# XiaRho/MADM

Hardware: NVIDIA B200
Metric: UNet feature-extract images/s @512^2 (VAE-enc + q-sample + SD-1.4 UNet+LoRA taps + projections) (higher is better)
Workload: dtype fp16

## Files before the change

### include/madm_b200.h

```cpp
#ifndef MADM_B200_H_
#define MADM_B200_H_

#include <stddef.h>
#include <stdint.h>

#ifdef __cplusplus
extern "C" {
#endif

#define MADM_VERSION 100

enum {
  MADM_OK = 0,
  MADM_EINVAL = -1,
  MADM_ENOTFOUND = -2,
  MADM_ECUDA = -3,
  MADM_ESTATE = -4,
  MADM_ENOMEM = -5
};

#define MADM_DTYPE_BF16 0
#define MADM_DTYPE_FP16 1

typedef struct madm_ctx madm_ctx;
typedef void* madm_stream;

typedef struct madm_tensor {
  const char* name;
  const void* data;
  int32_t ndim;
  int64_t shape[4];
} madm_tensor;

int madm_version(void);
const char* madm_last_error(const madm_ctx* ctx);

int madm_create(madm_ctx** out, int device);
int madm_destroy(madm_ctx* ctx);

int madm_set_compute_dtype(madm_ctx* ctx, int32_t dtype);
int madm_get_compute_dtype(const madm_ctx* ctx);

#define MADM_VARIANT_BASE 0
#define MADM_VARIANT_S0 1
int madm_set_variant(madm_ctx* ctx, int32_t variant);
int madm_get_variant(const madm_ctx* ctx);

int madm_set_tensors(madm_ctx* ctx, const madm_tensor* named, int32_t n);

size_t madm_packed_bytes(madm_ctx* ctx);

int madm_pack_weights(madm_ctx* ctx, void* packed, const char* adapter, float lora_alpha_over_r, int32_t lora_only,
                      madm_stream stream);

#define MADM_STAGE_VAE 1
#define MADM_STAGE_UNET 2
#define MADM_STAGE_PROJ 4
#define MADM_STAGE_ALL 7
#define MADM_STAGE_HEAD 8
#define MADM_STAGE_DEC 16
#define MADM_STAGE_ALL_S0 23

size_t madm_workspace_bytes(madm_ctx* ctx, int32_t B);
size_t madm_workspace_bytes_head(madm_ctx* ctx, int32_t B, int32_t head_h, int32_t head_w);

#define MADM_FLAG_IMG_NORMALISED 1
#define MADM_FLAG_OUT_FP16 4
typedef struct madm_extract_args {
  int32_t B;
  int32_t stages;
  int32_t ema;
  int32_t flags;
  const float* img;
  const float* cond_inputs;
  const float* cond_emb;
  const int64_t* timesteps;
  const float* shared_noise;
  const float* noisy_latents_in;
  float* out[4];
  float* latents;
  float* noisy_latents;
  float* taps[4];
  const void* packed;
  void* workspace;
  size_t workspace_bytes;
  int32_t* range_flag;
  float* logits;
  float* unet_sample;
  float* decoded;
  float* decoded_raw;
  int32_t head_h, head_w;
  const void* packed_dgrad;
  const char* train_adapter;
  float train_lora_scale;
  float train_loss_scale;
} madm_extract_args;

int madm_extract(madm_ctx* ctx, const madm_extract_args* args, madm_stream stream);

#define MADM_KIND_GEMM 0
#define MADM_KIND_ATTENTION 1
#define MADM_KIND_GROUPNORM 2
#define MADM_KIND_LAYERNORM 3
#define MADM_KIND_ELEMENTWISE 4
#define MADM_NUM_KINDS 5
typedef struct madm_profile {
  struct { char name[32]; int32_t launches; double ms; double flops; double bytes; double exec_flops; } kind[MADM_NUM_KINDS];
} madm_profile;
int madm_set_profiling(madm_ctx* ctx, int32_t on);
int madm_get_profile(madm_ctx* ctx, madm_profile* out);
int madm_get_profile_stages(madm_ctx* ctx, int32_t stage_mask, madm_profile* out);

int madm_launch_count(madm_ctx* ctx, int32_t B, int32_t stages);

typedef struct madm_gemm_seg {
  const void* a;
  int32_t Bt, H, W, C, ld, ntaps;
  int8_t dx[9], dy[9];
  int32_t b_off[9];
} madm_gemm_seg;

typedef struct madm_gemm_args {
  madm_gemm_seg seg[2];
  int32_t nseg, M, N, Nw, ldw;
  const void* w;
  const float* bias;
  const float* rowbias;
  int32_t rows_per_img, ld_rowbias;
  const float* residual;
  int32_t ldr;
  float* out_f32; int32_t ldo32;
  void* out_bf16; int32_t ldo16;
  int32_t act;
  float alpha;
  int32_t bn;
  int32_t dtype;
  float* colstats;
  int32_t stat_rows;
  int32_t mt;
  int32_t s2d_H, s2d_W;
  int32_t pair;
  int32_t res16;
} madm_gemm_args;

int madm_op_gemm(const madm_gemm_args* a, madm_stream stream);
int madm_op_groupnorm(const void* x0, int32_t C0, const void* x1, int32_t C1, int32_t B, int32_t HW,
                      int32_t in16 , const float* gamma,
                      const float* beta, float eps, int32_t act, float* stats_scratch ,
                      void* y_bf16, void* raw_bf16, int32_t dtype, madm_stream stream);
int madm_op_groupnorm_from_colstats(const void* x, int32_t C, int32_t B, int32_t HW, int32_t in16, const float* colstats,
                                    int32_t stat_rows, const float* gamma, const float* beta, float eps, int32_t act,
                                    float* scratch , void* y_bf16, int32_t dtype, madm_stream stream);
int madm_op_groupnorm_scratch_floats(int32_t B, int32_t HW, int32_t C);
int madm_op_layernorm(const void* x, int32_t in16 , int32_t M, int32_t C, const float* gamma,
                      const float* beta, float eps, void* y_bf16, int32_t dtype, madm_stream stream);
int madm_op_softmax_rows(const float* s, int32_t R, int32_t L, void* p_bf16, int32_t dtype, madm_stream stream);
int madm_op_attention(const void* q, int32_t ldq, const void* k, int32_t ldk, const void* v, int32_t ldv, void* o, int32_t ldo,
                      int32_t B, int32_t heads, int32_t d, int32_t Nq, int32_t Nk, int64_t q_bstride, int64_t kv_bstride,
                      int64_t o_bstride, float scale, int32_t dtype, int32_t impl ,
                      madm_stream stream);
int madm_op_pack_linear(const float* w, int32_t N, int32_t K, const float* lora_a, const float* lora_b, int32_t r, float scale,
                        void* out_bf16, int32_t ldo, int32_t dtype, madm_stream stream);
int madm_op_pack_conv(const float* w, int32_t N, int32_t C, int32_t taps, int32_t Cpad, void* out_bf16, int32_t ldo,
                      int32_t dtype, madm_stream stream);
int madm_op_pack_conv_dgrad(const float* w, int32_t Cout, int32_t Cin, int32_t taps, int32_t CoPad, void* out_bf16, int32_t ldo, int32_t dtype,
                            madm_stream stream);
int madm_op_pack_linear_dgrad(const float* w, int32_t N, int32_t K, const float* lora_a, const float* lora_b, int32_t r, float scale,
                              void* out_bf16, int32_t ldo, int32_t dtype, madm_stream stream);
int madm_op_pack_geglu(const float* w, const float* bias, int32_t C4, int32_t K, void* out_bf16, float* out_bias,
                       int32_t dtype, madm_stream stream);
int madm_op_space_to_depth(const float* x, int32_t B, int32_t H, int32_t W, int32_t C, void* out_bf16, int32_t dtype,
                           madm_stream stream);
int madm_op_nchw_to_nhwc16(const float* x, int32_t B, int32_t C, int32_t HW, void* out16, int32_t dtype, madm_stream stream);
int madm_op_bilinear_resize(const void* src16, int32_t B, int32_t Hs, int32_t Ws, int32_t C, void* dst16, int32_t Hd, int32_t Wd,
                            int32_t dst_pitch, int32_t dtype, madm_stream stream);
int madm_op_depthwise3x3(const void* src16, int32_t B, int32_t H, int32_t W, int32_t C, int32_t dilation, const float* w9 ,
                         const float* shift , void* dst16, int32_t dtype, madm_stream stream);
int madm_op_pseudo_labels(const float* logits , int32_t B, int32_t C, int32_t h, int32_t w, int32_t H, int32_t W, float threshold,
                          int32_t ignore_top, int64_t* label , float* prob , float* weight ,
                          int32_t* count , madm_stream stream);
int madm_op_class_mask(const int64_t* label, int64_t n, const int64_t* classes, int32_t k, int64_t* mask, madm_stream stream);
int madm_op_one_mix(const int64_t* mask, int64_t n, const int64_t* label_a, const int64_t* label_b, int64_t* label_out ,
                    const float* weight_a, const float* weight_b, float* weight_out , madm_stream stream);
int madm_op_preprocess_image(const float* src , int32_t planes, int32_t Hs, int32_t Ws, int32_t Hr, int32_t Wr, int32_t Hd,
                             int32_t Wd, float* dst , madm_stream stream);
int madm_op_image_mix(const int64_t* mask , const float* a , const float* b, int32_t C, int64_t HW, float* out,
                      madm_stream stream);
int madm_op_color_jitter(const float* in, int32_t B, int64_t HW, const int32_t* order, const float* factors, const float* mean, const float* stdv,
                         float* out, madm_stream stream);
int madm_op_gaussian_blur(const float* src , int32_t planes, int32_t H, int32_t W, int32_t ky, int32_t kx, float sigma_y,
                          float sigma_x, float* tmp , float* dst, madm_stream stream);
int madm_op_ema_update(float* const* ema, const float* const* param, const int64_t* numel, int32_t n, float alpha, float one_minus_alpha,
                       madm_stream stream);
int madm_op_grad_norm_scratch_floats(int32_t n);
int madm_op_grad_norm(const float* const* grad, const int64_t* numel, int32_t n, float* scratch, float* out_norm, madm_stream stream);
int madm_op_adamw_step(float* const* param, const float* const* grad, float* const* exp_avg, float* const* exp_avg_sq, const int64_t* numel,
                       int32_t n, double lr, double beta1, double beta2, double eps, double weight_decay, int32_t step, const float* grad_norm,
                       float max_norm, madm_stream stream);
int madm_op_slide_merge(const float* feats, int32_t nwin, int32_t n, int32_t C, int32_t hf, int32_t wf, const int32_t* wins, int32_t Hf,
                        int32_t Wf, float* out, madm_stream stream);
int madm_op_upsample2x(const float* x, int32_t B, int32_t H, int32_t W, int32_t C, void* out_bf16, int32_t dtype,
                       madm_stream stream);
int madm_op_image_im2col(const float* img, int32_t B, int32_t H, int32_t W, void* out_bf16, int32_t* range_flag,
                         int32_t dtype, madm_stream stream);
int madm_op_gn_add_relu_nchw(const float* a, const float* ga, const float* ba, const float* s, const float* gs, const float* bs,
                             int32_t has_shortcut_norm, float eps, int32_t B, int32_t HW, int32_t C, float* stats_scratch,
                             float* out_nchw, madm_stream stream);

#define MADM_FLAG_TRAIN 2
int madm_set_grad_tensors(madm_ctx* ctx, const madm_tensor* named, int32_t n);
size_t madm_dgrad_packed_bytes(madm_ctx* ctx);
int madm_pack_dgrad_weights(madm_ctx* ctx, void* packed_dgrad, const char* adapter, float lora_alpha_over_r, int32_t trainable_only,
                            madm_stream stream);
size_t madm_train_workspace_bytes(madm_ctx* ctx, int32_t B, const char* adapter);
typedef struct madm_backward_args {
  int32_t B;
  int32_t reserved;
  const float* dout[4];
  const float* out[4];
  const float* cond_emb;
  float* d_cond_inputs;
  float* d_cond_emb;
  const char* adapter;
  float lora_alpha_over_r;
  float loss_scale;
  const void* packed;
  const void* packed_dgrad;
  void* workspace;
  size_t workspace_bytes;
} madm_backward_args;
int madm_backward(madm_ctx* ctx, const madm_backward_args* args, madm_stream stream);
int madm_backward_launch_count(madm_ctx* ctx, int32_t B);

int madm_op_groupnorm_bwd_scratch_floats(int32_t B, int32_t HW, int32_t C);
int madm_op_groupnorm_bwd(const void* x0, int32_t C0, const void* x1, int32_t C1, int32_t B, int32_t HW, int32_t in16, const float* stats,
                          const float* gamma, const float* beta, float eps, int32_t act, const void* dy16, const float* extra, float* scratch,
                          void* out16, float* dx0, int32_t acc0, float* dx1, int32_t acc1, float* dgamma, float* dbeta, int32_t dtype,
                          madm_stream stream);
int madm_op_layernorm_bwd(const float* x, int32_t M, int32_t C, const float* gamma, float eps, const void* dy16, float* dx, int32_t accumulate,
                          int32_t dtype, madm_stream stream);
int madm_op_geglu_fwd(const void* raw16, int64_t M, int32_t H, void* out16, int32_t dtype, madm_stream stream);
int madm_op_geglu_bwd(const void* raw16, const void* dout16, int64_t M, int32_t H, void* draw16, int32_t dtype, madm_stream stream);
int64_t madm_op_attention_bwd_scratch_floats(int32_t B, int32_t heads, int32_t d, int32_t Nq, int32_t Nk);
int madm_op_attention_bwd(const void* q, int32_t ldq, const void* k, int32_t ldk, const void* v, int32_t ldv, const void* o, int32_t ldo,
                          const void* dout, int32_t lddo, void* dq, int32_t lddq, void* dk, int32_t lddk, void* dv, int32_t lddv, int32_t B,
                          int32_t heads, int32_t d, int32_t Nq, int32_t Nk, int64_t q_bs, int64_t kv_bs, int64_t o_bs, int64_t do_bs, int64_t dq_bs,
                          int64_t dkv_bs, float scale, float* scratch, int32_t dtype, madm_stream stream);
int64_t madm_op_wgrad_scratch_floats(int32_t M, int32_t N, int32_t K, int32_t taps);
int madm_op_wgrad(const void* dy16, int32_t lda, const void* x16, int32_t ldb, int32_t M, int32_t N, int32_t K, int32_t taps, int32_t Bimg, int32_t H,
                  int32_t W, float alpha, float* out, int32_t transpose_out, float* scratch, int32_t dtype, madm_stream stream);
int64_t madm_op_lora_grads_scratch_floats(int32_t M, int32_t N, int32_t K);
int madm_op_lora_grads(const void* x16, int32_t ldx, const void* dy16, int32_t ldy, const void* a16, const void* bt16, int32_t M, int32_t N, int32_t K,
                       float alpha, float* gA, float* gB, float* scratch, int32_t dtype, madm_stream stream);
int madm_op_colsum_per_image(const void* x16, int32_t B, int32_t HW, int32_t C, float* out, int32_t ldo, int32_t dtype, madm_stream stream);
int madm_op_zero_stuff2x(const void* x16, int32_t B, int32_t h, int32_t w, int32_t C, void* out16, madm_stream stream);
int madm_op_sum2x2(const float* x, int32_t B, int32_t h, int32_t w, int32_t C, float* out, int32_t accumulate, madm_stream stream);
int madm_op_relu_bwd_nchw(const float* dout, const float* out, int32_t B, int32_t C, int32_t HW, float scale, void* dz16, int32_t dtype,
                          madm_stream stream);

#ifdef __cplusplus
}
#endif
#endif
```

### madm_b200/_lib.py

```python
import ctypes as C
import os
from typing import Optional

_HERE = os.path.dirname(os.path.abspath(__file__))
LIB_PATH = os.environ.get("MADM_B200_LIB") or os.path.join(_HERE, "libmadm_b200.so")

MADM_OK = 0
STAGE_VAE, STAGE_UNET, STAGE_PROJ, STAGE_ALL = 1, 2, 4, 7
STAGE_HEAD = 8
STAGE_DEC, STAGE_ALL_S0 = 16, 23
VARIANT_BASE, VARIANT_S0 = 0, 1
FLAG_IMG_NORMALISED = 1
FLAG_TRAIN = 2
FLAG_OUT_FP16 = 4
ACT_NONE, ACT_SILU, ACT_GEGLU, ACT_RELU = 0, 1, 2, 3
DTYPE_BF16, DTYPE_FP16 = 0, 1

c_void_p, c_int, c_int32, c_int64, c_float, c_size_t, c_char_p = (
    C.c_void_p, C.c_int, C.c_int32, C.c_int64, C.c_float, C.c_size_t, C.c_char_p)


class MadmTensor(C.Structure):
    _fields_ = [("name", c_char_p), ("data", c_void_p), ("ndim", c_int32), ("shape", c_int64 * 4)]


class MadmExtractArgs(C.Structure):
    _fields_ = [
        ("B", c_int32), ("stages", c_int32), ("ema", c_int32), ("flags", c_int32),
        ("img", c_void_p), ("cond_inputs", c_void_p), ("cond_emb", c_void_p), ("timesteps", c_void_p),
        ("shared_noise", c_void_p), ("noisy_latents_in", c_void_p),
        ("out", c_void_p * 4),
        ("latents", c_void_p), ("noisy_latents", c_void_p), ("taps", c_void_p * 4),
        ("packed", c_void_p), ("workspace", c_void_p), ("workspace_bytes", c_size_t),
        ("range_flag", c_void_p), ("logits", c_void_p),
        ("unet_sample", c_void_p), ("decoded", c_void_p), ("decoded_raw", c_void_p),
        ("head_h", c_int32), ("head_w", c_int32),
        ("packed_dgrad", c_void_p), ("train_adapter", c_char_p), ("train_lora_scale", c_float), ("train_loss_scale", c_float),
    ]


class MadmBackwardArgs(C.Structure):
    _fields_ = [
        ("B", c_int32), ("reserved", c_int32),
        ("dout", c_void_p * 4), ("out", c_void_p * 4), ("cond_emb", c_void_p),
        ("d_cond_inputs", c_void_p), ("d_cond_emb", c_void_p),
        ("adapter", c_char_p), ("lora_alpha_over_r", c_float), ("loss_scale", c_float),
        ("packed", c_void_p), ("packed_dgrad", c_void_p), ("workspace", c_void_p), ("workspace_bytes", c_size_t),
    ]


class _MadmProfileKind(C.Structure):
    _fields_ = [("name", C.c_char * 32), ("launches", c_int32), ("ms", C.c_double), ("flops", C.c_double), ("bytes", C.c_double),
                ("exec_flops", C.c_double)]


class MadmProfile(C.Structure):
    _fields_ = [("kind", _MadmProfileKind * 5)]


class MadmGemmSeg(C.Structure):
    _fields_ = [("a", c_void_p), ("Bt", c_int32), ("H", c_int32), ("W", c_int32), ("C", c_int32), ("ld", c_int32),
                ("ntaps", c_int32), ("dx", C.c_int8 * 9), ("dy", C.c_int8 * 9), ("b_off", c_int32 * 9)]


class MadmGemmArgs(C.Structure):
    _fields_ = [
        ("seg", MadmGemmSeg * 2), ("nseg", c_int32), ("M", c_int32), ("N", c_int32), ("Nw", c_int32), ("ldw", c_int32),
        ("w", c_void_p), ("bias", c_void_p), ("rowbias", c_void_p), ("rows_per_img", c_int32), ("ld_rowbias", c_int32),
        ("residual", c_void_p), ("ldr", c_int32), ("out_f32", c_void_p), ("ldo32", c_int32),
        ("out_bf16", c_void_p), ("ldo16", c_int32), ("act", c_int32), ("alpha", c_float), ("bn", c_int32), ("dtype", c_int32),
        ("colstats", c_void_p), ("stat_rows", c_int32), ("mt", c_int32), ("s2d_H", c_int32), ("s2d_W", c_int32), ("pair", c_int32), ("res16", c_int32),
    ]


SYMBOLS = {
    "madm_version": (c_int, []),
    "madm_last_error": (c_char_p, [c_void_p]),
    "madm_create": (c_int, [C.POINTER(c_void_p), c_int]),
    "madm_destroy": (c_int, [c_void_p]),
    "madm_set_compute_dtype": (c_int, [c_void_p, c_int32]),
    "madm_get_compute_dtype": (c_int, [c_void_p]),
    "madm_set_variant": (c_int, [c_void_p, c_int32]),
    "madm_get_variant": (c_int, [c_void_p]),
    "madm_set_tensors": (c_int, [c_void_p, C.POINTER(MadmTensor), c_int32]),
    "madm_packed_bytes": (c_size_t, [c_void_p]),
    "madm_pack_weights": (c_int, [c_void_p, c_void_p, c_char_p, c_float, c_int32, c_void_p]),
    "madm_workspace_bytes": (c_size_t, [c_void_p, c_int32]),
    "madm_workspace_bytes_head": (c_size_t, [c_void_p, c_int32, c_int32, c_int32]),
    "madm_extract": (c_int, [c_void_p, C.POINTER(MadmExtractArgs), c_void_p]),
    "madm_set_grad_tensors": (c_int, [c_void_p, C.POINTER(MadmTensor), c_int32]),
    "madm_dgrad_packed_bytes": (c_size_t, [c_void_p]),
    "madm_pack_dgrad_weights": (c_int, [c_void_p, c_void_p, c_char_p, c_float, c_int32, c_void_p]),
    "madm_train_workspace_bytes": (c_size_t, [c_void_p, c_int32, c_char_p]),
    "madm_backward": (c_int, [c_void_p, C.POINTER(MadmBackwardArgs), c_void_p]),
    "madm_backward_launch_count": (c_int, [c_void_p, c_int32]),
    "madm_launch_count": (c_int, [c_void_p, c_int32, c_int32]),
    "madm_set_profiling": (c_int, [c_void_p, c_int32]),
    "madm_get_profile": (c_int, [c_void_p, C.POINTER(MadmProfile)]),
    "madm_get_profile_stages": (c_int, [c_void_p, c_int32, C.POINTER(MadmProfile)]),
    "madm_op_gemm": (c_int, [C.POINTER(MadmGemmArgs), c_void_p]),
    "madm_op_groupnorm": (c_int, [c_void_p, c_int32, c_void_p, c_int32, c_int32, c_int32, c_int32, c_void_p, c_void_p, c_float,
                                  c_int32, c_void_p, c_void_p, c_void_p, c_int32, c_void_p]),
    "madm_op_groupnorm_scratch_floats": (c_int, [c_int32, c_int32, c_int32]),
    "madm_op_groupnorm_from_colstats": (c_int, [c_void_p, c_int32, c_int32, c_int32, c_int32, c_void_p, c_int32, c_void_p, c_void_p,
                                                c_float, c_int32, c_void_p, c_void_p, c_int32, c_void_p]),
    "madm_op_layernorm": (c_int, [c_void_p, c_int32, c_int32, c_int32, c_void_p, c_void_p, c_float, c_void_p, c_int32, c_void_p]),
    "madm_op_softmax_rows": (c_int, [c_void_p, c_int32, c_int32, c_void_p, c_int32, c_void_p]),
    "madm_op_attention": (c_int, [c_void_p, c_int32, c_void_p, c_int32, c_void_p, c_int32, c_void_p, c_int32, c_int32,
                                  c_int32, c_int32, c_int32, c_int32, c_int64, c_int64, c_int64, c_float, c_int32, c_int32, c_void_p]),
    "madm_op_pack_linear": (c_int, [c_void_p, c_int32, c_int32, c_void_p, c_void_p, c_int32, c_float, c_void_p, c_int32,
                                    c_int32, c_void_p]),
    "madm_op_pack_conv": (c_int, [c_void_p, c_int32, c_int32, c_int32, c_int32, c_void_p, c_int32, c_int32, c_void_p]),
    "madm_op_pack_conv_dgrad": (c_int, [c_void_p, c_int32, c_int32, c_int32, c_int32, c_void_p, c_int32, c_int32, c_void_p]),
    "madm_op_pack_linear_dgrad": (c_int, [c_void_p, c_int32, c_int32, c_void_p, c_void_p, c_int32, c_float, c_void_p, c_int32, c_int32, c_void_p]),
    "madm_op_pack_geglu": (c_int, [c_void_p, c_void_p, c_int32, c_int32, c_void_p, c_void_p, c_int32, c_void_p]),
    "madm_op_space_to_depth": (c_int, [c_void_p, c_int32, c_int32, c_int32, c_int32, c_void_p, c_int32, c_void_p]),
    "madm_op_nchw_to_nhwc16": (c_int, [c_void_p, c_int32, c_int32, c_int32, c_void_p, c_int32, c_void_p]),
    "madm_op_bilinear_resize": (c_int, [c_void_p, c_int32, c_int32, c_int32, c_int32, c_void_p, c_int32, c_int32, c_int32, c_int32, c_void_p]),
    "madm_op_depthwise3x3": (c_int, [c_void_p, c_int32, c_int32, c_int32, c_int32, c_int32, c_void_p, c_void_p, c_void_p, c_int32, c_void_p]),
    "madm_op_pseudo_labels": (c_int, [c_void_p, c_int32, c_int32, c_int32, c_int32, c_int32, c_int32, c_float, c_int32, c_void_p, c_void_p,
                                      c_void_p, c_void_p, c_void_p]),
    "madm_op_class_mask": (c_int, [c_void_p, c_int64, c_void_p, c_int32, c_void_p, c_void_p]),
    "madm_op_one_mix": (c_int, [c_void_p, c_int64, c_void_p, c_void_p, c_void_p, c_void_p, c_void_p, c_void_p, c_void_p]),
    "madm_op_preprocess_image": (c_int, [c_void_p, c_int32, c_int32, c_int32, c_int32, c_int32, c_int32, c_int32, c_void_p, c_void_p]),
    "madm_op_image_mix": (c_int, [c_void_p, c_void_p, c_void_p, c_int32, c_int64, c_void_p, c_void_p]),
    "madm_op_color_jitter": (c_int, [c_void_p, c_int32, c_int64, c_void_p, c_void_p, c_void_p, c_void_p, c_void_p, c_void_p]),
    "madm_op_gaussian_blur": (c_int, [c_void_p, c_int32, c_int32, c_int32, c_int32, c_int32, c_float, c_float, c_void_p, c_void_p, c_void_p]),
    "madm_op_ema_update": (c_int, [c_void_p, c_void_p, c_void_p, c_int32, c_float, c_float, c_void_p]),
    "madm_op_grad_norm_scratch_floats": (c_int, [c_int32]),
    "madm_op_grad_norm": (c_int, [c_void_p, c_void_p, c_int32, c_void_p, c_void_p, c_void_p]),
    "madm_op_adamw_step": (c_int, [c_void_p, c_void_p, c_void_p, c_void_p, c_void_p, c_int32, C.c_double, C.c_double, C.c_double, C.c_double,
                                   C.c_double, c_int32, c_void_p, c_float, c_void_p]),
    "madm_op_slide_merge": (c_int, [c_void_p, c_int32, c_int32, c_int32, c_int32, c_int32, c_void_p, c_int32, c_int32, c_void_p, c_void_p]),
    "madm_op_upsample2x": (c_int, [c_void_p, c_int32, c_int32, c_int32, c_int32, c_void_p, c_int32, c_void_p]),
    "madm_op_image_im2col": (c_int, [c_void_p, c_int32, c_int32, c_int32, c_void_p, c_void_p, c_int32, c_void_p]),
    "madm_op_groupnorm_bwd_scratch_floats": (c_int, [c_int32, c_int32, c_int32]),
    "madm_op_groupnorm_bwd": (c_int, [c_void_p, c_int32, c_void_p, c_int32, c_int32, c_int32, c_int32, c_void_p, c_void_p, c_void_p, c_float, c_int32,
                                      c_void_p, c_void_p, c_void_p, c_void_p, c_void_p, c_int32, c_void_p, c_int32, c_void_p, c_void_p, c_int32, c_void_p]),
    "madm_op_layernorm_bwd": (c_int, [c_void_p, c_int32, c_int32, c_void_p, c_float, c_void_p, c_void_p, c_int32, c_int32, c_void_p]),
    "madm_op_geglu_fwd": (c_int, [c_void_p, c_int64, c_int32, c_void_p, c_int32, c_void_p]),
    "madm_op_geglu_bwd": (c_int, [c_void_p, c_void_p, c_int64, c_int32, c_void_p, c_int32, c_void_p]),
    "madm_op_attention_bwd_scratch_floats": (c_int64, [c_int32, c_int32, c_int32, c_int32, c_int32]),
    "madm_op_attention_bwd": (c_int, [c_void_p, c_int32, c_void_p, c_int32, c_void_p, c_int32, c_void_p, c_int32, c_void_p, c_int32, c_void_p, c_int32,
                                      c_void_p, c_int32, c_void_p, c_int32, c_int32, c_int32, c_int32, c_int32, c_int32, c_int64, c_int64, c_int64,
                                      c_int64, c_int64, c_int64, c_float, c_void_p, c_int32, c_void_p]),
    "madm_op_wgrad_scratch_floats": (c_int64, [c_int32, c_int32, c_int32, c_int32]),
    "madm_op_wgrad": (c_int, [c_void_p, c_int32, c_void_p, c_int32, c_int32, c_int32, c_int32, c_int32, c_int32, c_int32, c_int32, c_float, c_void_p,
                              c_int32, c_void_p, c_int32, c_void_p]),
    "madm_op_lora_grads_scratch_floats": (c_int64, [c_int32, c_int32, c_int32]),
    "madm_op_lora_grads": (c_int, [c_void_p, c_int32, c_void_p, c_int32, c_void_p, c_void_p, c_int32, c_int32, c_int32, c_float, c_void_p, c_void_p,
                                   c_void_p, c_int32, c_void_p]),
    "madm_op_colsum_per_image": (c_int, [c_void_p, c_int32, c_int32, c_int32, c_void_p, c_int32, c_int32, c_void_p]),
    "madm_op_zero_stuff2x": (c_int, [c_void_p, c_int32, c_int32, c_int32, c_int32, c_void_p, c_void_p]),
    "madm_op_sum2x2": (c_int, [c_void_p, c_int32, c_int32, c_int32, c_int32, c_void_p, c_int32, c_void_p]),
    "madm_op_relu_bwd_nchw": (c_int, [c_void_p, c_void_p, c_int32, c_int32, c_int32, c_float, c_void_p, c_int32, c_void_p]),
    "madm_op_gn_add_relu_nchw": (c_int, [c_void_p, c_void_p, c_void_p, c_void_p, c_void_p, c_void_p, c_int32, c_float,
                                         c_int32, c_int32, c_int32, c_void_p, c_void_p, c_void_p]),
}

_lib: Optional[C.CDLL] = None


class MadmError(RuntimeError):
    pass


def load() -> C.CDLL:
    global _lib
    if _lib is not None:
        return _lib
    if not os.path.exists(LIB_PATH):
        raise MadmError(
            f"{LIB_PATH} not found: build it with `python -c 'import __graft_entry__ as g; g.build()'` "
            "(nvcc, sm_100a). madm_b200 has no CPU / PyTorch fallback.")
    lib = C.CDLL(LIB_PATH)
    for name, (res, args) in SYMBOLS.items():
        fn = getattr(lib, name)
        fn.restype = res
        fn.argtypes = args
    _lib = lib
    return lib


def check(rc: int, ctx=None, what: str = ""):
    if rc != MADM_OK:
        lib = load()
        msg = lib.madm_last_error(ctx)
        raise MadmError(f"{what} failed ({rc}): {msg.decode() if msg else ''}")
```

### madm_b200/csrc/api_ops.cu

```cuda
#include "../../include/madm_b200.h"
#include "api_internal.h"
#include "kernels.h"

#include <string.h>

using namespace madm;

namespace madm {
static thread_local char g_err[512] = "";
void set_global_error(const char* msg) {
  strncpy(g_err, msg ? msg : "", sizeof(g_err) - 1);
  g_err[sizeof(g_err) - 1] = 0;
}
const char* global_error() { return g_err; }
}

static int fail(const char* e) {
  set_global_error(e);
  return MADM_EINVAL;
}
#define RUN(expr)                      \
  do {                                 \
    const char* _e = (expr);           \
    if (_e) return fail(_e);           \
    return MADM_OK;                    \
  } while (0)

extern "C" {

int madm_op_gemm(const madm_gemm_args* a, madm_stream stream) {
  if (!a) return fail("madm_op_gemm: null args");
  GemmDesc d;
  d.nseg = a->nseg;
  for (int s = 0; s < 2; ++s) {
    const madm_gemm_seg& g = a->seg[s];
    GemmASeg& t = d.seg[s];
    t.ptr = g.a; t.Bt = g.Bt; t.H = g.H; t.W = g.W; t.C = g.C; t.ld = g.ld; t.ntaps = g.ntaps;
    for (int i = 0; i < 9; ++i) { t.dx[i] = g.dx[i]; t.dy[i] = g.dy[i]; t.b_off[i] = g.b_off[i]; }
  }
  d.M = a->M; d.N = a->N; d.w = a->w; d.Nw = a->Nw; d.ldw = a->ldw;
  d.bias = a->bias; d.rowbias = a->rowbias; d.rows_per_img = a->rows_per_img; d.ld_rowbias = a->ld_rowbias;
  d.residual = a->residual; d.ldr = a->ldr;
  d.out_f32 = a->out_f32; d.ldo32 = a->ldo32; d.out_bf16 = a->out_bf16; d.ldo16 = a->ldo16;
  d.act = a->act; d.alpha = a->alpha; d.bn = a->bn; d.fp16 = a->dtype == MADM_DTYPE_FP16;
  d.colstats = a->colstats; d.stat_rows = a->stat_rows ? a->stat_rows : 32; d.mt = a->mt; d.s2d_H = a->s2d_H; d.s2d_W = a->s2d_W; d.pair = a->pair; d.res16 = a->res16;
  GemmLaunch L;
  if (const char* e = gemm_prepare(d, &L)) return fail(e);
  RUN(gemm_launch(L, static_cast<cudaStream_t>(stream)));
}

int madm_op_groupnorm(const void* x0, int32_t C0, const void* x1, int32_t C1, int32_t B, int32_t HW, int32_t in16, const float* gamma,
                      const float* beta, float eps, int32_t act, float* stats, void* y, void* raw, int32_t dtype, madm_stream stream) {
  cudaStream_t st = static_cast<cudaStream_t>(stream);
  const int f16 = dtype == MADM_DTYPE_FP16;
  if (const char* e = groupnorm_stats(x0, C0, x1, C1, B, HW, in16, f16, stats, st)) return fail(e);
  RUN(groupnorm_apply(x0, C0, x1, C1, B, HW, in16, stats, 0, gamma, beta, eps, act, y, raw, f16, st));
}

int madm_op_layernorm(const void* x, int32_t in16, int32_t M, int32_t C, const float* gamma, const float* beta, float eps, void* y,
                      int32_t dtype, madm_stream stream) {
  RUN(layernorm(x, in16, M, C, gamma, beta, eps, y, dtype == MADM_DTYPE_FP16, static_cast<cudaStream_t>(stream)));
}

int madm_op_softmax_rows(const float* s, int32_t R, int32_t L, void* p, int32_t dtype, madm_stream stream) {
  RUN(softmax_rows(s, R, L, p, dtype == MADM_DTYPE_FP16, static_cast<cudaStream_t>(stream)));
}

int madm_op_attention(const void* q, int32_t ldq, const void* k, int32_t ldk, const void* v, int32_t ldv, void* o, int32_t ldo,
                      int32_t B, int32_t heads, int32_t d, int32_t Nq, int32_t Nk, int64_t q_bs, int64_t kv_bs, int64_t o_bs,
                      float scale, int32_t dtype, int32_t impl, madm_stream stream) {
  if (impl != 0) return fail("madm_op_attention: impl must be 0 (the mma.sync kernel of round 1 was removed from the library)");
  FaLaunch L;
  if (const char* e = flash_attention_tc_prepare(q, ldq, k, ldk, v, ldv, o, ldo, B, heads, d, Nq, Nk, q_bs, kv_bs, o_bs, scale,
                                                 dtype == MADM_DTYPE_FP16, &L))
    return fail(e);
  RUN(flash_attention_tc_launch(L, static_cast<cudaStream_t>(stream)));
}

int madm_op_pack_linear(const float* w, int32_t N, int32_t K, const float* la, const float* lb, int32_t r, float scale, void* out,
                        int32_t ldo, int32_t dtype, madm_stream stream) {
  RUN(pack_linear_weight(w, N, K, la, lb, r, scale, ldo ? ldo : K, out, dtype == MADM_DTYPE_FP16, static_cast<cudaStream_t>(stream)));
}

int madm_op_pack_conv(const float* w, int32_t N, int32_t C, int32_t taps, int32_t Cpad, void* out, int32_t ldo, int32_t dtype,
                      madm_stream stream) {
  const int Kpad = taps * Cpad;
  RUN(pack_conv_weight(w, N, C, taps, Cpad, Kpad, ldo ? ldo : Kpad, out, dtype == MADM_DTYPE_FP16, static_cast<cudaStream_t>(stream)));
}

int madm_op_pack_conv_dgrad(const float* w, int32_t Cout, int32_t Cin, int32_t taps, int32_t CoPad, void* out, int32_t ldo, int32_t dtype,
                            madm_stream stream) {
  const int Kpad = taps * CoPad;
  RUN(pack_conv_dgrad_weight(w, Cout, Cin, taps, CoPad, Kpad, ldo ? ldo : Kpad, out, dtype == MADM_DTYPE_FP16, static_cast<cudaStream_t>(stream)));
}

int madm_op_pack_linear_dgrad(const float* w, int32_t N, int32_t K, const float* lora_a, const float* lora_b, int32_t r, float scale, void* out,
                              int32_t ldo, int32_t dtype, madm_stream stream) {
  RUN(pack_linear_dgrad_weight(w, N, K, lora_a, lora_b, r, scale, ldo ? ldo : N, out, dtype == MADM_DTYPE_FP16, static_cast<cudaStream_t>(stream)));
}

int madm_op_pack_geglu(const float* w, const float* bias, int32_t C4, int32_t K, void* out, float* out_bias, int32_t dtype,
                       madm_stream stream) {
  RUN(pack_geglu_weight(w, bias, C4, K, out, out_bias, dtype == MADM_DTYPE_FP16, static_cast<cudaStream_t>(stream)));
}

int madm_op_space_to_depth(const float* x, int32_t B, int32_t H, int32_t W, int32_t C, void* out, int32_t dtype, madm_stream stream) {
  RUN(space_to_depth(x, B, H, W, C, out, dtype == MADM_DTYPE_FP16, static_cast<cudaStream_t>(stream)));
}

int madm_op_upsample2x(const float* x, int32_t B, int32_t H, int32_t W, int32_t C, void* out, int32_t dtype, madm_stream stream) {
  RUN(upsample_nearest2x(x, B, H, W, C, out, dtype == MADM_DTYPE_FP16, static_cast<cudaStream_t>(stream)));
}

int madm_op_nchw_to_nhwc16(const float* x, int32_t B, int32_t C, int32_t HW, void* out, int32_t dtype, madm_stream stream) {
  RUN(nchw_to_nhwc16(x, B, C, HW, out, dtype == MADM_DTYPE_FP16, static_cast<cudaStream_t>(stream)));
}

int madm_op_bilinear_resize(const void* src, int32_t B, int32_t Hs, int32_t Ws, int32_t C, void* dst, int32_t Hd, int32_t Wd, int32_t ldd,
                            int32_t dtype, madm_stream stream) {
  RUN(bilinear_resize_nhwc16(src, B, Hs, Ws, C, dst, Hd, Wd, ldd, dtype == MADM_DTYPE_FP16, static_cast<cudaStream_t>(stream)));
}

int madm_op_depthwise3x3(const void* src, int32_t B, int32_t H, int32_t W, int32_t C, int32_t dilation, const float* w9, const float* shift,
                         void* dst, int32_t dtype, madm_stream stream) {
  RUN(depthwise3x3_nhwc16(src, B, H, W, C, dilation, w9, shift, dst, dtype == MADM_DTYPE_FP16, static_cast<cudaStream_t>(stream)));
}

int madm_op_pseudo_labels(const float* logits, int32_t B, int32_t C, int32_t h, int32_t w, int32_t H, int32_t W, float threshold,
                          int32_t ignore_top, int64_t* label, float* prob, float* weight, int32_t* count, madm_stream stream) {
  RUN(pseudo_labels(logits, B, C, h, w, H, W, threshold, ignore_top, label, prob, weight, count, static_cast<cudaStream_t>(stream)));
}

int madm_op_class_mask(const int64_t* label, int64_t n, const int64_t* classes, int32_t k, int64_t* mask, madm_stream stream) {
  RUN(class_mask(label, long(n), classes, k, mask, static_cast<cudaStream_t>(stream)));
}

int madm_op_one_mix(const int64_t* mask, int64_t n, const int64_t* label_a, const int64_t* label_b, int64_t* label_out, const float* weight_a,
                    const float* weight_b, float* weight_out, madm_stream stream) {
  RUN(one_mix(mask, long(n), label_a, label_b, label_out, weight_a, weight_b, weight_out, static_cast<cudaStream_t>(stream)));
}

int madm_op_ema_update(float* const* ema, const float* const* param, const int64_t* numel, int32_t n, float alpha, float one_minus_alpha,
                       madm_stream stream) {
  if (!ema || !param || !numel || n < 1) return fail("madm_op_ema_update: null argument");
  RUN(ema_update(ema, param, reinterpret_cast<const long*>(numel), n, alpha, one_minus_alpha, static_cast<cudaStream_t>(stream)));
}

int madm_op_grad_norm_scratch_floats(int32_t n) { return grad_norm_scratch_floats(n); }

int madm_op_grad_norm(const float* const* grad, const int64_t* numel, int32_t n, float* scratch, float* out_norm, madm_stream stream) {
  if (!grad || !numel || !scratch || !out_norm || n < 1) return fail("madm_op_grad_norm: null argument");
  RUN(grad_norm(grad, reinterpret_cast<const long*>(numel), n, scratch, out_norm, static_cast<cudaStream_t>(stream)));
}

int madm_op_adamw_step(float* const* param, const float* const* grad, float* const* exp_avg, float* const* exp_avg_sq, const int64_t* numel,
                       int32_t n, double lr, double beta1, double beta2, double eps, double weight_decay, int32_t step, const float* grad_norm,
                       float max_norm, madm_stream stream) {
  if (!param || !grad || !exp_avg || !exp_avg_sq || !numel || n < 1) return fail("madm_op_adamw_step: null argument");
  RUN(adamw_step(param, grad, exp_avg, exp_avg_sq, reinterpret_cast<const long*>(numel), n, lr, beta1, beta2, eps, weight_decay, step, grad_norm,
                 max_norm, static_cast<cudaStream_t>(stream)));
}

int madm_op_preprocess_image(const float* src, int32_t planes, int32_t Hs, int32_t Ws, int32_t Hr, int32_t Wr, int32_t Hd, int32_t Wd, float* dst,
                             madm_stream stream) {
  if (!src || !dst) return fail("madm_op_preprocess_image: null argument");
  RUN(resize_bilinear_nchw(src, planes, Hs, Ws, Hr, Wr, Hd, Wd, dst, static_cast<cudaStream_t>(stream)));
}

int madm_op_image_mix(const int64_t* mask, const float* a, const float* b, int32_t C, int64_t HW, float* out, madm_stream stream) {
  if (!mask || !a || !b || !out) return fail("madm_op_image_mix: null argument");
  RUN(image_mix(mask, a, b, C, long(HW), out, static_cast<cudaStream_t>(stream)));
}

int madm_op_color_jitter(const float* in, int32_t B, int64_t HW, const int32_t* order, const float* factors, const float* mean, const float* stdv,
                         float* out, madm_stream stream) {
  if (!in || !order || !factors || !out) return fail("madm_op_color_jitter: null argument");
  RUN(color_jitter(in, B, long(HW), order, factors, mean, stdv, out, static_cast<cudaStream_t>(stream)));
}

int madm_op_gaussian_blur(const float* src, int32_t planes, int32_t H, int32_t W, int32_t ky, int32_t kx, float sigma_y, float sigma_x, float* tmp,
                          float* dst, madm_stream stream) {
  if (!src || !tmp || !dst) return fail("madm_op_gaussian_blur: null argument");
  RUN(gaussian_blur(src, planes, H, W, ky, kx, sigma_y, sigma_x, tmp, dst, static_cast<cudaStream_t>(stream)));
}

int madm_op_slide_merge(const float* feats, int32_t nwin, int32_t n, int32_t C, int32_t hf, int32_t wf, const int32_t* wins, int32_t Hf, int32_t Wf,
                        float* out, madm_stream stream) {
  RUN(slide_merge(feats, nwin, n, C, hf, wf, wins, Hf, Wf, out, static_cast<cudaStream_t>(stream)));
}

int madm_op_image_im2col(const float* img, int32_t B, int32_t H, int32_t W, void* out, int32_t* range_flag, int32_t dtype,
                         madm_stream stream) {
  RUN(image_im2col(img, B, H, W, out, range_flag, dtype == MADM_DTYPE_FP16, static_cast<cudaStream_t>(stream)));
}

int madm_op_groupnorm_from_colstats(const void* x, int32_t C, int32_t B, int32_t HW, int32_t in16, const float* colstats, int32_t stat_rows,
                                    const float* gamma, const float* beta, float eps, int32_t act, float* scratch , void* y,
                                    int32_t dtype, madm_stream stream) {
  cudaStream_t st = static_cast<cudaStream_t>(stream);
  const int f16 = dtype == MADM_DTYPE_FP16;
  if (HW % stat_rows != 0) return fail("groupnorm_from_colstats: HW must be a multiple of stat_rows");
  if (stat_rows != 32) return fail("groupnorm_from_colstats: stat_rows must be 32");
  const int nb = HW / stat_rows;
  if (const char* e = groupnorm_colstats_reduce(colstats, C, nullptr, 0, B, nb, scratch, st)) return fail(e);
  RUN(groupnorm_apply(x, C, nullptr, 0, B, HW, in16, scratch, groupnorm_colstats_chunks(nb), gamma, beta, eps, act, y, nullptr, f16, st));
}

int madm_op_groupnorm_scratch_floats(int32_t B, int32_t HW, int32_t C) {
  return int(size_t(2) * B * groupnorm_slabs(HW, C) * 64 + size_t(2) * B * 64);
}

int madm_op_gn_add_relu_nchw(const float* a, const float* ga, const float* ba, const float* s, const float* gs, const float* bs,
                             int32_t has_shortcut_norm, float eps, int32_t B, int32_t HW, int32_t C, float* stats, float* out,
                             madm_stream stream) {
  cudaStream_t st = static_cast<cudaStream_t>(stream);
  const size_t per = size_t(B) * groupnorm_slabs(HW, C) * 64;
  float* pa = stats;
  float* ps = stats + per;
  float* st_a = stats + 2 * per;
  float* st_s = st_a + size_t(B) * 64;
  if (const char* e = groupnorm_stats(a, C, nullptr, 0, B, HW, 0, 0, pa, st)) return fail(e);
  if (const char* e = groupnorm_finalize(pa, B, HW, C, st_a, st)) return fail(e);
  if (has_shortcut_norm) {
    if (const char* e = groupnorm_stats(s, C, nullptr, 0, B, HW, 0, 0, ps, st)) return fail(e);
    if (const char* e = groupnorm_finalize(ps, B, HW, C, st_s, st)) return fail(e);
  }
  RUN(gn_add_relu_nchw(a, st_a, ga, ba, s, has_shortcut_norm ? st_s : nullptr, gs, bs, eps, B, HW, C, out, st));
}

int madm_op_groupnorm_bwd_scratch_floats(int32_t B, int32_t HW, int32_t C) {
  return int(size_t(B) * groupnorm_bwd_slabs(HW) * C * 2 + size_t(B) * 64 + size_t(B) * C * 2);
}
int madm_op_groupnorm_bwd(const void* x0, int32_t C0, const void* x1, int32_t C1, int32_t B, int32_t HW, int32_t in16, const float* stats,
                          const float* gamma, const float* beta, float eps, int32_t act, const void* dy16, const float* extra, float* scratch,
                          void* out16, float* dx0, int32_t acc0, float* dx1, int32_t acc1, float* dgamma, float* dbeta, int32_t dtype,
                          madm_stream stream) {
  const int C = C0 + C1;
  float* partial = scratch;
  float* coef = partial + size_t(B) * groupnorm_bwd_slabs(HW) * C * 2;
  float* chan = coef + size_t(B) * 64;
  RUN(groupnorm_bwd(x0, C0, x1, C1, B, HW, in16, stats, gamma, beta, eps, act, dy16, dtype == MADM_DTYPE_FP16, partial, coef, chan, extra, out16, dx0,
                    acc0, dx1, acc1, dgamma, dbeta, 1.0f, static_cast<cudaStream_t>(stream)));
}
int madm_op_layernorm_bwd(const float* x, int32_t M, int32_t C, const float* gamma, float eps, const void* dy16, float* dx, int32_t accumulate,
                          int32_t dtype, madm_stream stream) {
  RUN(layernorm_bwd(x, M, C, gamma, eps, dy16, dtype == MADM_DTYPE_FP16, dx, accumulate, static_cast<cudaStream_t>(stream)));
}
int madm_op_geglu_fwd(const void* raw16, int64_t M, int32_t H, void* out16, int32_t dtype, madm_stream stream) {
  RUN(geglu_fwd(raw16, long(M), H, out16, dtype == MADM_DTYPE_FP16, static_cast<cudaStream_t>(stream)));
}
int madm_op_geglu_bwd(const void* raw16, const void* dout16, int64_t M, int32_t H, void* draw16, int32_t dtype, madm_stream stream) {
  RUN(geglu_bwd(raw16, dout16, long(M), H, draw16, dtype == MADM_DTYPE_FP16, static_cast<cudaStream_t>(stream)));
}
int64_t madm_op_attention_bwd_scratch_floats(int32_t B, int32_t heads, int32_t d, int32_t Nq, int32_t Nk) {
  return int64_t(attention_bwd_scratch_floats(B, heads, d, Nq, Nk));
}
int madm_op_attention_bwd(const void* q, int32_t ldq, const void* k, int32_t ldk, const void* v, int32_t ldv, const void* o, int32_t ldo,
                          const void* dout, int32_t lddo, void* dq, int32_t lddq, void* dk, int32_t lddk, void* dv, int32_t lddv, int32_t B,
                          int32_t heads, int32_t d, int32_t Nq, int32_t Nk, int64_t q_bs, int64_t kv_bs, int64_t o_bs, int64_t do_bs, int64_t dq_bs,
                          int64_t dkv_bs, float scale, float* scratch, int32_t dtype, madm_stream stream) {
  RUN(attention_bwd(q, ldq, k, ldk, v, ldv, o, ldo, dout, lddo, dq, lddq, dk, lddk, dv, lddv, B, heads, d, Nq, Nk, long(q_bs), long(kv_bs), long(kv_bs),
                    long(o_bs), long(do_bs), long(dq_bs), long(dkv_bs), long(dkv_bs), scale, scratch, dtype == MADM_DTYPE_FP16,
                    static_cast<cudaStream_t>(stream)));
}
int64_t madm_op_wgrad_scratch_floats(int32_t M, int32_t N, int32_t K, int32_t taps) { return int64_t(wgrad_scratch_floats(M, N, K, taps)); }
int madm_op_wgrad(const void* dy16, int32_t lda, const void* x16, int32_t ldb, int32_t M, int32_t N, int32_t K, int32_t taps, int32_t Bimg, int32_t H,
                  int32_t W, float alpha, float* out, int32_t transpose_out, float* scratch, int32_t dtype, madm_stream stream) {
  long so_n = K, so_k = 1, so_tap = 0;
  if (taps == 9) { so_n = long(K) * 9; so_k = 9; so_tap = 1; }
  else if (transpose_out) { so_n = 1; so_k = N; }
  RUN(wgrad(dy16, lda, x16, ldb, M, N, K, taps, Bimg, H, W, alpha, out, so_n, so_k, so_tap, scratch, dtype == MADM_DTYPE_FP16,
            static_cast<cudaStream_t>(stream)));
}
int64_t madm_op_lora_grads_scratch_floats(int32_t M, int32_t N, int32_t K) { return lora_grads_supported(N, K) ? int64_t(lora_grads_scratch_floats(M, N, K)) : -1; }
int madm_op_lora_grads(const void* x16, int32_t ldx, const void* dy16, int32_t ldy, const void* a16, const void* bt16, int32_t M, int32_t N, int32_t K,
                       float alpha, float* gA, float* gB, float* scratch, int32_t dtype, madm_stream stream) {
  RUN(lora_grads(x16, ldx, dy16, ldy, a16, bt16, M, N, K, alpha, gA, gB, scratch, dtype == MADM_DTYPE_FP16, static_cast<cudaStream_t>(stream)));
}
int madm_op_colsum_per_image(const void* x16, int32_t B, int32_t HW, int32_t C, float* out, int32_t ldo, int32_t dtype, madm_stream stream) {
  RUN(colsum_per_image(x16, B, HW, C, dtype == MADM_DTYPE_FP16, out, ldo, static_cast<cudaStream_t>(stream)));
}
int madm_op_zero_stuff2x(const void* x16, int32_t B, int32_t h, int32_t w, int32_t C, void* out16, madm_stream stream) {
  RUN(zero_stuff2x(x16, B, h, w, C, out16, static_cast<cudaStream_t>(stream)));
}
int madm_op_sum2x2(const float* x, int32_t B, int32_t h, int32_t w, int32_t C, float* out, int32_t accumulate, madm_stream stream) {
  RUN(sum2x2(x, B, h, w, C, out, accumulate, static_cast<cudaStream_t>(stream)));
}
int madm_op_relu_bwd_nchw(const float* dout, const float* out, int32_t B, int32_t C, int32_t HW, float scale, void* dz16, int32_t dtype,
                          madm_stream stream) {
  RUN(relu_bwd_nchw_to_nhwc16(dout, out, B, C, HW, scale, dz16, dtype == MADM_DTYPE_FP16, static_cast<cudaStream_t>(stream)));
}

}
```

### madm_b200/csrc/attention_tc.cu

```cuda
#include "cvt.cuh"
#include "kernels.h"
#include "launch.cuh"
#include "ptx.cuh"

#include <mutex>
#include <stdio.h>

namespace madm {

static constexpr int FA_BM = 128;
static constexpr int FA_BN = 128;
static constexpr int FA_TILE = 128 * 128;

template <int D, int NQT>
struct FaCfg {
  static constexpr int KC = (D + 63) / 64;
  static constexpr int DV = (D + 15) / 16 * 16;
  static constexpr int KSTEPS = (D + 15) / 16;
  static constexpr bool REG_S = D <= 80;
  static constexpr bool ONES = REG_S && DV > D;
  static constexpr int NSB = REG_S ? 1 : 2;
  static constexpr bool P_TMEM = ONES && NQT == 2;
  static constexpr int Q_BYTES = NQT * KC * FA_TILE;
  static constexpr int KV_BYTES = KC * FA_TILE;
  static constexpr int P_BYTES = P_TMEM ? 0 : NQT * 2 * FA_TILE;
  static constexpr int STAGES = (Q_BYTES + P_BYTES + 4 * KV_BYTES + 2048 <= 227 * 1024) ? 2 : 1;
  static constexpr size_t SMEM = Q_BYTES + 2 * STAGES * KV_BYTES + P_BYTES + 1024 + 512;
  static constexpr int S_COLS = NQT * NSB * 128;
  static constexpr int P_COLS = P_TMEM ? NQT * 64 : 0;
  static constexpr int O_BASE = S_COLS + P_COLS;
  static constexpr int O_STRIDE = (DV + 31) / 32 * 32;
  static constexpr int TMEM_NEED = O_BASE + NQT * O_STRIDE;
  static constexpr int TMEM_COLS = TMEM_NEED <= 256 ? 256 : 512;
  static constexpr int THREADS = 32 * (1 + NQT) + NQT * 128;
  static_assert(TMEM_NEED <= 512, "TMEM budget");
  static_assert(SMEM <= 227 * 1024, "smem budget");
};

struct FaParams {
  CUtensorMap tmQ, tmK, tmV;
  uint16_t* O;
  int ldo;
  long o_bs;
  int Nq, Nk;
  float scale_log2;
  int fp16;
  float* lse;
};

__device__ __forceinline__ float fa_ex2(float x) {
  float y;
  asm("ex2.approx.ftz.f32 %0, %1;" : "=f"(y) : "f"(x));
  return y;
}

template <int D, int NQT, bool FP16>
__global__ void __launch_bounds__(FaCfg<D, NQT>::THREADS, 1) fa_tc_kernel(const __grid_constant__ FaParams p) {
  using C = FaCfg<D, NQT>;
  extern __shared__ uint8_t smem_raw[];
  const uint32_t base = (smem_u32(smem_raw) + 1023u) & ~1023u;
  const uint32_t sQ = base;
  const uint32_t sK = sQ + C::Q_BYTES;
  const uint32_t sV = sK + C::STAGES * C::KV_BYTES;
  const uint32_t sP = sV + C::STAGES * C::KV_BYTES;
  const uint32_t sBar = sP + C::P_BYTES;
  const uint32_t q_full = sBar;
  auto k_full = [&](int s) { return sBar + 8u * (1 + s); };
  auto k_empty = [&](int s) { return sBar + 8u * (3 + s); };
  auto v_full = [&](int s) { return sBar + 8u * (5 + s); };
  auto v_empty = [&](int s) { return sBar + 8u * (7 + s); };
  auto gbar = [&](int g, int i) { return sBar + 8u * (9 + g * 8 + i); };
  auto s_full = [&](int g, int a) { return gbar(g, a); };
  auto s_empty = [&](int g, int a) { return gbar(g, 2 + a); };
  auto pv_go = [&](int g) { return gbar(g, 4); };
  auto pv_done = [&](int g) { return gbar(g, 5); };
  const uint32_t tmem_slot = sBar + 8u * (9 + 16);
  volatile uint32_t* tmem_slot_ptr = reinterpret_cast<volatile uint32_t*>(smem_raw + (tmem_slot - smem_u32(smem_raw)));

  const int warp = threadIdx.x >> 5, lane = threadIdx.x & 31;
  const int q0 = blockIdx.x * (FA_BM * NQT), h = blockIdx.y, b = blockIdx.z;
  const int ntiles = (p.Nk + FA_BN - 1) / FA_BN;

  if (warp == 0 && lane == 0) {
    prefetch_tmap(&p.tmQ); prefetch_tmap(&p.tmK); prefetch_tmap(&p.tmV);
    mbar_init(q_full, 1);
    for (int s = 0; s < 2; ++s) {
      mbar_init(k_full(s), 1); mbar_init(k_empty(s), NQT); mbar_init(v_full(s), 1); mbar_init(v_empty(s), NQT);
    }
    for (int g = 0; g < NQT; ++g) {
      for (int a = 0; a < 2; ++a) { mbar_init(s_full(g, a), 1); mbar_init(s_empty(g, a), 4); }
      mbar_init(pv_go(g), 4); mbar_init(pv_done(g), 1);
    }
    fence_mbar_init();
  }
  if (warp == 1) {
    tmem_alloc(tmem_slot, C::TMEM_COLS);
    tmem_relinquish();
  }
  tc_fence_before();
  __syncthreads();
  tc_fence_after();
  const uint32_t tmem = *tmem_slot_ptr;
  pdl_trigger();
  pdl_wait();

  if (warp == 0) {
    if (elect_one()) {
      mbar_arrive_expect_tx(q_full, C::Q_BYTES);
#pragma unroll
      for (int g = 0; g < NQT; ++g)
#pragma unroll
        for (int kc = 0; kc < C::KC; ++kc)
          tma_load_4d(sQ + (g * C::KC + kc) * FA_TILE, &p.tmQ, q_full, kc * 64, h, q0 + g * FA_BM, b);
      int stage = 0;
      uint32_t phase = 0;
      for (int j = 0; j < ntiles; ++j) {
        mbar_wait(k_empty(stage), phase ^ 1u);
        mbar_arrive_expect_tx(k_full(stage), C::KV_BYTES);
#pragma unroll
        for (int kc = 0; kc < C::KC; ++kc) tma_load_4d(sK + stage * C::KV_BYTES + kc * FA_TILE, &p.tmK, k_full(stage), kc * 64, h, j * FA_BN, b);
        mbar_wait(v_empty(stage), phase ^ 1u);
        mbar_arrive_expect_tx(v_full(stage), C::KV_BYTES);
#pragma unroll
        for (int kc = 0; kc < C::KC; ++kc) tma_load_4d(sV + stage * C::KV_BYTES + kc * FA_TILE, &p.tmV, v_full(stage), kc * 64, h, j * FA_BN, b);
        if (++stage == C::STAGES) { stage = 0; phase ^= 1u; }
      }
    }
  } else if (warp <= NQT) {
    if (elect_one()) {
      const int g = warp - 1;
      const uint32_t idesc_s = make_idesc_16(FA_BM, FA_BN, FP16 ? 1 : 0);
      const uint32_t idesc_o = make_idesc_16(FA_BM, C::DV, FP16 ? 1 : 0) | (1u << 16);
      uint64_t qd[C::KSTEPS], kd[C::STAGES][C::KSTEPS], vd[C::STAGES], pd[2];
#pragma unroll
      for (int ks = 0; ks < C::KSTEPS; ++ks) {
        const int kc = ks >> 2, k = ks & 3;
        qd[ks] = make_smem_desc_sw128(sQ + (g * C::KC + kc) * FA_TILE) + uint64_t(2 * k);
#pragma unroll
        for (int st = 0; st < C::STAGES; ++st) kd[st][ks] = make_smem_desc_sw128(sK + st * C::KV_BYTES + kc * FA_TILE) + uint64_t(2 * k);
      }
#pragma unroll
      for (int st = 0; st < C::STAGES; ++st) vd[st] = make_smem_desc_sw128_mn(sV + st * C::KV_BYTES, FA_TILE);
      pd[0] = make_smem_desc_sw128(sP + (g * 2) * FA_TILE);
      pd[1] = make_smem_desc_sw128(sP + (g * 2 + 1) * FA_TILE);
      const uint32_t tmem_og = tmem + C::O_BASE + g * C::O_STRIDE;
      const uint32_t tmem_pg = tmem + C::S_COLS + g * 64;
      auto issue_s = [&](int j) {
        const int stage = j % C::STAGES;
        const int sb = j % C::NSB;
        mbar_wait(k_full(stage), (j / C::STAGES) & 1);
        mbar_wait(s_empty(g, sb), ((j / C::NSB) & 1) ^ 1u);
        tc_fence_after();
        const uint32_t ts = tmem + uint32_t((g * C::NSB + sb) * 128);
#pragma unroll
        for (int ks = 0; ks < C::KSTEPS; ++ks) umma_bf16_ss(ts, qd[ks], stage == 0 ? kd[0][ks] : kd[C::STAGES - 1][ks], idesc_s, ks != 0);
        umma_commit(s_full(g, sb));
        umma_commit(k_empty(stage));
      };
      mbar_wait(q_full, 0);
      issue_s(0);
      for (int j = 0; j < ntiles; ++j) {
        if (j + 1 < ntiles) issue_s(j + 1);
        const int stage = j % C::STAGES;
        int keys = p.Nk - j * FA_BN;
        if (keys > FA_BN) keys = FA_BN;
        const int ksteps = (keys + 15) >> 4;
        mbar_wait(pv_go(g), j & 1);
        tc_fence_after();
        const uint64_t vds = stage == 0 ? vd[0] : vd[C::STAGES - 1];
#pragma unroll
        for (int kk = 0; kk < FA_BN / 16; ++kk) {
          if (kk < ksteps) {
            const uint64_t bd = vds + uint64_t(kk * (2048 >> 4));
            if constexpr (C::P_TMEM) umma_f16_ts(tmem_og, tmem_pg + kk * 8, bd, idesc_o, kk != 0);
            else umma_bf16_ss(tmem_og, pd[kk >> 2] + uint64_t(2 * (kk & 3)), bd, idesc_o, kk != 0);
          }
        }
        umma_commit(pv_done(g));
        umma_commit(v_empty(stage));
      }
    }
  } else {
    const int g = (warp - (1 + NQT)) >> 2;
    const int q = warp & 3;
    const int row = q * 32 + lane;
    const uint32_t lane_base = uint32_t(q * 32) << 16;
    const uint32_t sPg = sP + uint32_t(g * 2) * FA_TILE;
    const uint32_t tmem_o = tmem + lane_base + C::O_BASE + g * C::O_STRIDE;
    const uint32_t tmem_p = tmem + lane_base + C::S_COLS + g * 64;
    const float sl = p.scale_log2;
    constexpr int fp16 = FP16 ? 1 : 0;
    constexpr int OC = C::ONES ? D + 1 : D;
    float o_acc[C::DV];
#pragma unroll
    for (int i = 0; i < C::DV; ++i) o_acc[i] = 0.f;
    float m_run = -INFINITY, l_run = 0.f, corr_prev = 1.f;
    uint32_t r[32];

    auto o_update = [&](float corr) {
      tc_fence_after();
      constexpr int OB = (C::DV % 48 == 0) ? 48 : 32;
#pragma unroll
      for (int c0 = 0; c0 < C::DV; c0 += OB) {
        uint32_t ro[OB];
        __syncwarp();
        if (c0 + 0 < C::DV) tmem_ld16_at<0>(tmem_o + c0, ro);
        if (c0 + 16 < C::DV) tmem_ld16_at<16>(tmem_o + c0 + 16, ro);
        if constexpr (OB == 48) { if (c0 + 32 < C::DV) tmem_ld16_at<32>(tmem_o + c0 + 32, ro); }
        tmem_ld_wait();
#pragma unroll
        for (int i = 0; i < OB; ++i)
          if (c0 + i < OC) o_acc[c0 + i] = fmaf(o_acc[c0 + i], corr, __uint_as_float(ro[i]));
      }
      tc_fence_before();
    };

    for (int j = 0; j < ntiles; ++j) {
      const int sb = j % C::NSB;
      mbar_wait(s_full(g, sb), (j / C::NSB) & 1);
      tc_fence_after();
      const uint32_t ts = tmem + lane_base + uint32_t((g * C::NSB + sb) * 128);
      const int kvalid = p.Nk - j * FA_BN;
      const bool ragged = kvalid < FA_BN;
      float corr, rs = 0.f;
      if constexpr (C::REG_S && C::P_TMEM) {
        uint32_t sc[4][32];
        __syncwarp();
#pragma unroll
        for (int c = 0; c < 4; ++c) tmem_ld32(ts + c * 32, sc[c]);
        tmem_ld_wait();
        tc_fence_before();
        __syncwarp();
        if (lane == 0) mbar_arrive(s_empty(g, sb));
        if (ragged) {
#pragma unroll
          for (int c = 0; c < 4; ++c)
#pragma unroll
            for (int i = 0; i < 32; ++i)
              if (c * 32 + i >= kvalid) sc[c][i] = 0xff800000u;
        }
        float mx0 = m_run, mx1 = -INFINITY, mx2 = -INFINITY, mx3 = -INFINITY;
#pragma unroll
        for (int i = 0; i < 32; ++i) {
          mx0 = fmaxf(mx0, __uint_as_float(sc[0][i]));
          mx1 = fmaxf(mx1, __uint_as_float(sc[1][i]));
          mx2 = fmaxf(mx2, __uint_as_float(sc[2][i]));
          mx3 = fmaxf(mx3, __uint_as_float(sc[3][i]));
        }
        const float mx = fmaxf(fmaxf(mx0, mx1), fmaxf(mx2, mx3));
        corr = fa_ex2((m_run - mx) * sl);
        m_run = mx;
        const float ms = -mx * sl;
        {
          const int stage = j % C::STAGES;
          mbar_wait(v_full(stage), (j / C::STAGES) & 1);
          if constexpr (C::ONES) {
            const uint32_t addr = sV + stage * C::KV_BYTES + uint32_t(D >> 6) * FA_TILE + uint32_t(row) * 128 +
                                  uint32_t((((D & 63) >> 3) ^ (row & 7)) << 4) + uint32_t((D & 7) * 2);
            const uint16_t one = FP16 ? 0x3C00 : 0x3F80;
            asm volatile("st.shared.u16 [%0], %1;" ::"r"(addr), "h"(one) : "memory");
          }
        }
        float rs1 = 0.f;
#pragma unroll
        for (int c = 0; c < 4; ++c) {
          uint32_t pk[16];
#pragma unroll
          for (int i = 0; i < 32; i += 2) {
            const float p0 = fa_ex2(fmaf(__uint_as_float(sc[c][i]), sl, ms));
            const float p1 = fa_ex2(fmaf(__uint_as_float(sc[c][i + 1]), sl, ms));
            pk[i >> 1] = pack2_16(p0, p1, fp16);
            if constexpr (!C::ONES) { rs += p0; rs1 += p1; }
          }
          if (c == 0) {
            if (j > 0) mbar_wait(pv_done(g), (j - 1) & 1);
            if constexpr (C::P_TMEM) { tc_fence_after(); __syncwarp(); }
          }
          if constexpr (C::P_TMEM) {
            tmem_st16(tmem_p + c * 16, pk);
          } else {
            const uint32_t chunk_base = sPg + uint32_t(c >> 1) * FA_TILE + uint32_t(row) * 128;
            const int u0 = (c & 1) * 4;
#pragma unroll
            for (int u = 0; u < 4; ++u) {
              const uint32_t addr = chunk_base + uint32_t(((u0 + u) ^ (row & 7)) << 4);
              asm volatile("st.shared.v4.b32 [%0], {%1,%2,%3,%4};" ::"r"(addr), "r"(pk[4 * u]), "r"(pk[4 * u + 1]), "r"(pk[4 * u + 2]),
                           "r"(pk[4 * u + 3]) : "memory");
            }
          }
        }
        if constexpr (C::P_TMEM) { tmem_st_wait(); tc_fence_before(); }
        rs += rs1;
      } else if constexpr (C::REG_S) {
        uint32_t sa[32], sb2[32];
        float mx0 = m_run, mx1 = -INFINITY, mx2 = -INFINITY, mx3 = -INFINITY;
#pragma unroll
        for (int hlf = 0; hlf < 2; ++hlf) {
          __syncwarp();
          tmem_ld32(ts + hlf * 64, sa);
          tmem_ld32(ts + hlf * 64 + 32, sb2);
          tmem_ld_wait();
          if (ragged) {
#pragma unroll
            for (int i = 0; i < 32; ++i) {
              if (hlf * 64 + i >= kvalid) sa[i] = 0xff800000u;
              if (hlf * 64 + 32 + i >= kvalid) sb2[i] = 0xff800000u;
            }
          }
#pragma unroll
          for (int i = 0; i < 32; i += 2) {
            mx0 = fmaxf(mx0, __uint_as_float(sa[i]));
            mx1 = fmaxf(mx1, __uint_as_float(sa[i + 1]));
            mx2 = fmaxf(mx2, __uint_as_float(sb2[i]));
            mx3 = fmaxf(mx3, __uint_as_float(sb2[i + 1]));
          }
        }
        const float mx = fmaxf(fmaxf(mx0, mx1), fmaxf(mx2, mx3));
        corr = fa_ex2((m_run - mx) * sl);
        m_run = mx;
        const float ms = -mx * sl;
        {
          const int stage = j % C::STAGES;
          mbar_wait(v_full(stage), (j / C::STAGES) & 1);
          if constexpr (C::ONES) {
            const uint32_t addr = sV + stage * C::KV_BYTES + uint32_t(D >> 6) * FA_TILE + uint32_t(row) * 128 +
                                  uint32_t((((D & 63) >> 3) ^ (row & 7)) << 4) + uint32_t((D & 7) * 2);
            const uint16_t one = FP16 ? 0x3C00 : 0x3F80;
            asm volatile("st.shared.u16 [%0], %1;" ::"r"(addr), "h"(one) : "memory");
          }
        }
        float rs1 = 0.f;
        __syncwarp();
        tmem_ld32(ts, sa);
#pragma unroll
        for (int c = 0; c < 4; ++c) {
          uint32_t (&cur)[32] = (c & 1) ? sb2 : sa;
          uint32_t (&nxt)[32] = (c & 1) ? sa : sb2;
          tmem_ld_wait();
          if (c < 3) {
            __syncwarp();
            tmem_ld32(ts + (c + 1) * 32, nxt);
          } else {
            tc_fence_before();
            __syncwarp();
            if (lane == 0) mbar_arrive(s_empty(g, sb));
          }
          if (ragged) {
#pragma unroll
            for (int i = 0; i < 32; ++i)
              if (c * 32 + i >= kvalid) cur[i] = 0xff800000u;
          }
          uint32_t pk[16];
#pragma unroll
          for (int i = 0; i < 32; i += 2) {
            const float p0 = fa_ex2(fmaf(__uint_as_float(cur[i]), sl, ms));
            const float p1 = fa_ex2(fmaf(__uint_as_float(cur[i + 1]), sl, ms));
            pk[i >> 1] = pack2_16(p0, p1, fp16);
            if constexpr (!C::ONES) { rs += p0; rs1 += p1; }
          }
          if (c == 0 && j > 0) mbar_wait(pv_done(g), (j - 1) & 1);
          const uint32_t chunk_base = sPg + uint32_t(c >> 1) * FA_TILE + uint32_t(row) * 128;
          const int u0 = (c & 1) * 4;
#pragma unroll
          for (int u = 0; u < 4; ++u) {
            const uint32_t addr = chunk_base + uint32_t(((u0 + u) ^ (row & 7)) << 4);
            asm volatile("st.shared.v4.b32 [%0], {%1,%2,%3,%4};" ::"r"(addr), "r"(pk[4 * u]), "r"(pk[4 * u + 1]), "r"(pk[4 * u + 2]),
                         "r"(pk[4 * u + 3]) : "memory");
          }
        }
        rs += rs1;
      } else {
        float mx = m_run;
#pragma unroll 1
        for (int c = 0; c < FA_BN; c += 32) {
          __syncwarp();
          tmem_ld32(ts + c, r);
          tmem_ld_wait();
          if (c + 32 <= kvalid) {
#pragma unroll
            for (int i = 0; i < 32; ++i) mx = fmaxf(mx, __uint_as_float(r[i]));
          } else {
#pragma unroll
            for (int i = 0; i < 32; ++i)
              if (c + i < kvalid) mx = fmaxf(mx, __uint_as_float(r[i]));
          }
        }
        corr = fa_ex2((m_run - mx) * sl);
        m_run = mx;
        const float ms = -mx * sl;
        mbar_wait(v_full(j % C::STAGES), (j / C::STAGES) & 1);
        if (j > 0) mbar_wait(pv_done(g), (j - 1) & 1);
#pragma unroll 1
        for (int c = 0; c < FA_BN; c += 32) {
          __syncwarp();
          tmem_ld32(ts + c, r);
          tmem_ld_wait();
          uint32_t pk[16];
#pragma unroll
          for (int i = 0; i < 32; i += 2) {
            float p0 = fa_ex2(fmaf(__uint_as_float(r[i]), sl, ms));
            float p1 = fa_ex2(fmaf(__uint_as_float(r[i + 1]), sl, ms));
            if (c + i >= kvalid) p0 = 0.f;
            if (c + i + 1 >= kvalid) p1 = 0.f;
            rs += p0 + p1;
            pk[i >> 1] = pack2_16(p0, p1, fp16);
          }
          const uint32_t chunk_base = sPg + uint32_t(c >> 6) * FA_TILE + uint32_t(row) * 128;
          const int u0 = (c & 63) >> 3;
#pragma unroll
          for (int u = 0; u < 4; ++u) {
            const uint32_t addr = chunk_base + uint32_t(((u0 + u) ^ (row & 7)) << 4);
            asm volatile("st.shared.v4.b32 [%0], {%1,%2,%3,%4};" ::"r"(addr), "r"(pk[4 * u]), "r"(pk[4 * u + 1]), "r"(pk[4 * u + 2]),
                         "r"(pk[4 * u + 3]) : "memory");
          }
        }
        tc_fence_before();
        __syncwarp();
        if (lane == 0) mbar_arrive(s_empty(g, sb));
      }
      l_run = l_run * corr + rs;
      fence_proxy_async();
      if (j > 0) o_update(corr_prev);
      corr_prev = corr;
      tc_fence_before();
      __syncwarp();
      if (lane == 0) mbar_arrive(pv_go(g));
    }
    mbar_wait(pv_done(g), (ntiles - 1) & 1);
    o_update(corr_prev);
    const int m = q0 + g * FA_BM + row;
    if (m < p.Nq) {
      const float den = C::ONES ? o_acc[C::ONES ? D : 0] : l_run;
      const float inv = 1.0f / den;
      if (p.lse) p.lse[(size_t(b) * gridDim.y + h) * p.Nq + m] = (m_run * p.scale_log2 + log2f(den)) * 0.6931471805599453f;
      uint16_t* op = p.O + size_t(b) * p.o_bs + size_t(m) * p.ldo + h * D;
#pragma unroll
      for (int c = 0; c < D; c += 8) {
        uint4 v;
        v.x = pack2_16(o_acc[c] * inv, o_acc[c + 1] * inv, fp16);
        v.y = pack2_16(o_acc[c + 2] * inv, o_acc[c + 3] * inv, fp16);
        v.z = pack2_16(o_acc[c + 4] * inv, o_acc[c + 5] * inv, fp16);
        v.w = pack2_16(o_acc[c + 6] * inv, o_acc[c + 7] * inv, fp16);
        *reinterpret_cast<uint4*>(op + c) = v;
      }
    }
  }

  tc_fence_before();
  __syncthreads();
  if (warp == 1) {
    tc_fence_after();
    tmem_dealloc(tmem, C::TMEM_COLS);
  }
}

typedef CUresult (*EncodeTiledFn)(CUtensorMap*, CUtensorMapDataType, cuuint32_t, void*, const cuuint64_t*, const cuuint64_t*,
                                  const cuuint32_t*, const cuuint32_t*, CUtensorMapInterleave, CUtensorMapSwizzle,
                                  CUtensorMapL2promotion, CUtensorMapFloatOOBfill);
static EncodeTiledFn fa_encode_fn() {
  static EncodeTiledFn fn = nullptr;
  static std::once_flag once;
  std::call_once(once, [] {
    void* p = nullptr;
    cudaDriverEntryPointQueryResult qres;
    if (cudaGetDriverEntryPoint("cuTensorMapEncodeTiled", &p, cudaEnableDefault, &qres) == cudaSuccess && qres == cudaDriverEntryPointSuccess)
      fn = reinterpret_cast<EncodeTiledFn>(p);
  });
  return fn;
}

static const char* fa_map(CUtensorMap* tm, const void* ptr, int d, int heads, int ntok, int B, int ld, long bstride) {
  EncodeTiledFn fn = fa_encode_fn();
  if (!fn) return "cuTensorMapEncodeTiled unavailable";
  cuuint64_t dims[4] = {cuuint64_t(d), cuuint64_t(heads), cuuint64_t(ntok), cuuint64_t(B)};
  cuuint64_t strides[3] = {cuuint64_t(d) * 2, cuuint64_t(ld) * 2, cuuint64_t(bstride) * 2};
  if (B == 1) strides[2] = cuuint64_t(ntok) * ld * 2;
  cuuint32_t box[4] = {64, 1, 128, 1};
  cuuint32_t estr[4] = {1, 1, 1, 1};
  CUresult r = fn(tm, CU_TENSOR_MAP_DATA_TYPE_UINT16, 4, const_cast<void*>(ptr), dims, strides, box, estr, CU_TENSOR_MAP_INTERLEAVE_NONE,
                  CU_TENSOR_MAP_SWIZZLE_128B, CU_TENSOR_MAP_L2_PROMOTION_L2_256B, CU_TENSOR_MAP_FLOAT_OOB_FILL_NONE);
  if (r != CUDA_SUCCESS) {
    static thread_local char buf[128];
    snprintf(buf, sizeof(buf), "attention: cuTensorMapEncodeTiled failed (CUresult %d)", int(r));
    return buf;
  }
  return nullptr;
}

const char* flash_attention_tc_prepare(const void* q, int ldq, const void* k, int ldk, const void* v, int ldv, void* o, int ldo, int B,
                                       int heads, int d, int Nq, int Nk, long q_bs, long kv_bs, long o_bs, float scale, int fp16,
                                       FaLaunch* L, float* lse) {
  if (d != 40 && d != 80 && d != 160) return "attention: unsupported head dim (40, 80, 160)";
  if (ldq % 8 || ldk % 8 || ldv % 8 || ldo % 8 || q_bs % 8 || kv_bs % 8) return "attention: pitches must be multiples of 8 elements";
  if ((reinterpret_cast<uintptr_t>(q) | reinterpret_cast<uintptr_t>(k) | reinterpret_cast<uintptr_t>(v) | reinterpret_cast<uintptr_t>(o)) & 15)
    return "attention: pointers must be 16-byte aligned";
  if (Nq < 1 || Nk < 1) return "attention: empty problem";
  static_assert(sizeof(FaParams) <= sizeof(L->params), "FaLaunch::params too small");
  FaParams* p = reinterpret_cast<FaParams*>(L->params);
  if (const char* e = fa_map(&p->tmQ, q, d, heads, Nq, B, ldq, q_bs)) return e;
  if (const char* e = fa_map(&p->tmK, k, d, heads, Nk, B, ldk, kv_bs)) return e;
  if (const char* e = fa_map(&p->tmV, v, d, heads, Nk, B, ldv, kv_bs)) return e;
  p->O = reinterpret_cast<uint16_t*>(o);
  p->ldo = ldo; p->o_bs = o_bs; p->Nq = Nq; p->Nk = Nk;
  p->scale_log2 = scale * 1.4426950408889634f;
  p->fp16 = fp16;
  p->lse = lse;
  L->d = d;
  L->nqt = (d <= 80 && Nq >= 2 * FA_BM) ? 2 : 1;
  L->grid = dim3((Nq + FA_BM * L->nqt - 1) / (FA_BM * L->nqt), heads, B);
  return nullptr;
}

template <int D, int NQT, bool FP16>
static const char* fa_launch_t(const FaLaunch& L, cudaStream_t st) {
  using C = FaCfg<D, NQT>;
  static bool attr = false;
  if (!attr) {
    if (cudaFuncSetAttribute(fa_tc_kernel<D, NQT, FP16>, cudaFuncAttributeMaxDynamicSharedMemorySize, int(C::SMEM)) != cudaSuccess)
      return "attention: cudaFuncSetAttribute failed";
    attr = true;
  }
  if (launch_k(fa_tc_kernel<D, NQT, FP16>, L.grid, dim3(C::THREADS), C::SMEM, st, *reinterpret_cast<const FaParams*>(L.params)) != cudaSuccess)
    return "fa_tc launch failed";
  return cudaGetLastError() == cudaSuccess ? nullptr : "attention: launch failed";
}
template <int D, int NQT>
static const char* fa_launch_d(const FaLaunch& L, cudaStream_t st) {
  return reinterpret_cast<const FaParams*>(L.params)->fp16 ? fa_launch_t<D, NQT, true>(L, st) : fa_launch_t<D, NQT, false>(L, st);
}

const char* flash_attention_tc_launch(const FaLaunch& L, cudaStream_t st) {
  switch (L.d) {
    case 40: return L.nqt == 2 ? fa_launch_d<40, 2>(L, st) : fa_launch_d<40, 1>(L, st);
    case 80: return L.nqt == 2 ? fa_launch_d<80, 2>(L, st) : fa_launch_d<80, 1>(L, st);
    case 160: return fa_launch_d<160, 1>(L, st);
  }
  return "attention: unsupported head dim";
}

}
```

### madm_b200/ops.py

```python
import ctypes as C
from typing import Optional, Sequence

import torch

from . import _lib
from ._lib import MadmGemmArgs, MadmGemmSeg


def _ptr(t: Optional[torch.Tensor]):
    return None if t is None else C.c_void_p(t.data_ptr())


def _dt(dtype) -> int:
    if dtype == torch.float16:
        return _lib.DTYPE_FP16
    if dtype == torch.bfloat16:
        return _lib.DTYPE_BF16
    raise _lib.MadmError(f"operand dtype must be torch.float16 or torch.bfloat16, got {dtype}")


def _stream():
    return C.c_void_p(torch.cuda.current_stream().cuda_stream)


def taps_3x3():
    return [(kx - 1, ky - 1, 0) for ky in range(3) for kx in range(3)]


def taps_stride2(B: int, pad1: bool):
    out = []
    for ky in range(3):
        for kx in range(3):
            if pad1:
                py, dy = (0 if ky == 1 else 1), (-1 if ky == 0 else 0)
                px, dx = (0 if kx == 1 else 1), (-1 if kx == 0 else 0)
            else:
                py, dy = (1 if ky == 1 else 0), (1 if ky == 2 else 0)
                px, dx = (1 if kx == 1 else 0), (1 if kx == 2 else 0)
            out.append((dx, dy, (py * 2 + px) * B))
    return out


def make_seg(a: torch.Tensor, Bt: int, H: int, W: int, Cc: int, ld: int = 0, taps: Optional[Sequence] = None) -> MadmGemmSeg:
    s = MadmGemmSeg()
    s.a = a.data_ptr()
    s.Bt, s.H, s.W, s.C, s.ld = Bt, H, W, Cc, ld
    taps = taps or [(0, 0, 0)]
    s.ntaps = len(taps)
    for i, (dx, dy, bo) in enumerate(taps):
        s.dx[i], s.dy[i], s.b_off[i] = dx, dy, bo
    return s


def gemm(segs: Sequence[MadmGemmSeg], M: int, N: int, w: torch.Tensor, *, Nw: int = 0, ldw: int = 0,
         bias=None, rowbias=None, rows_per_img: int = 1, ld_rowbias: int = 0, residual=None, ldr: int = 0,
         out_f32=None, ldo32: int = 0, out_bf16=None, ldo16: int = 0, act: int = 0, alpha: float = 1.0, bn: int = 0,
         colstats=None, stat_rows: int = 0, mt: int = 0, s2d_hw=None, pair: int = 0):
    a = MadmGemmArgs()
    a.nseg = len(segs)
    for i, s in enumerate(segs):
        a.seg[i] = s
    a.M, a.N, a.Nw, a.ldw = M, N, Nw or N, ldw
    a.w = w.data_ptr()
    a.bias = bias.data_ptr() if bias is not None else None
    a.rowbias = rowbias.data_ptr() if rowbias is not None else None
    a.rows_per_img, a.ld_rowbias = rows_per_img, ld_rowbias
    a.residual = residual.data_ptr() if residual is not None else None
    a.ldr = ldr
    a.res16 = 1 if (residual is not None and residual.dtype != torch.float32) else 0
    a.out_f32 = out_f32.data_ptr() if out_f32 is not None else None
    a.ldo32 = ldo32
    a.out_bf16 = out_bf16.data_ptr() if out_bf16 is not None else None
    a.ldo16 = ldo16
    a.act, a.alpha, a.bn = act, alpha, bn
    a.dtype = _dt(w.dtype)
    a.colstats = colstats.data_ptr() if colstats is not None else None
    a.stat_rows = stat_rows
    a.mt = mt
    a.pair = pair
    if s2d_hw is not None:
        a.s2d_H, a.s2d_W = s2d_hw
    lib = _lib.load()
    _lib.check(lib.madm_op_gemm(C.byref(a), _stream()), None, "madm_op_gemm")


def groupnorm(x0, x1, B, HW, gamma, beta, eps, act, y, raw=None):
    lib = _lib.load()
    C0 = x0.shape[-1]
    C1 = x1.shape[-1] if x1 is not None else 0
    stats = torch.empty(lib.madm_op_groupnorm_scratch_floats(B, HW, C0 + C1), dtype=torch.float32, device=x0.device)
    in16 = 0 if x0.dtype == torch.float32 else 1
    _lib.check(lib.madm_op_groupnorm(_ptr(x0), C0, _ptr(x1), C1, B, HW, in16, _ptr(gamma), _ptr(beta), eps, act, _ptr(stats),
                                     _ptr(y), _ptr(raw), _dt(y.dtype), _stream()), None, "madm_op_groupnorm")
    return stats


def groupnorm_from_colstats(x, B, HW, colstats, stat_rows, gamma, beta, eps, act, y):
    lib = _lib.load()
    Cc = x.shape[-1]
    scratch = torch.empty(B * 32 * 64, dtype=torch.float32, device=x.device)
    in16 = 0 if x.dtype == torch.float32 else 1
    _lib.check(lib.madm_op_groupnorm_from_colstats(_ptr(x), Cc, B, HW, in16, _ptr(colstats), stat_rows, _ptr(gamma), _ptr(beta), eps, act,
                                                   _ptr(scratch), _ptr(y), _dt(y.dtype), _stream()), None, "madm_op_groupnorm_from_colstats")


def layernorm(x, gamma, beta, eps, y):
    lib = _lib.load()
    M, Cc = x.shape
    in16 = 0 if x.dtype == torch.float32 else 1
    _lib.check(lib.madm_op_layernorm(_ptr(x), in16, M, Cc, _ptr(gamma), _ptr(beta), eps, _ptr(y), _dt(y.dtype), _stream()), None, "madm_op_layernorm")


def softmax_rows(s, p):
    lib = _lib.load()
    R, L = s.shape
    _lib.check(lib.madm_op_softmax_rows(_ptr(s), R, L, _ptr(p), _dt(p.dtype), _stream()), None, "madm_op_softmax_rows")


def attention(q, ldq, k, ldk, v, ldv, o, ldo, B, heads, d, Nq, Nk, q_bs, kv_bs, o_bs, scale, impl=0):
    lib = _lib.load()
    _lib.check(lib.madm_op_attention(_ptr(q), ldq, _ptr(k), ldk, _ptr(v), ldv, _ptr(o), ldo, B, heads, d, Nq, Nk, q_bs, kv_bs,
                                     o_bs, scale, _dt(o.dtype), impl, _stream()), None, "madm_op_attention")


def pack_linear(w, lora_a=None, lora_b=None, scale=0.0, out=None, ldo=0, dtype=torch.float16):
    lib = _lib.load()
    N, K = w.shape
    r = lora_a.shape[0] if lora_a is not None else 0
    if out is None:
        out = torch.empty(N, K, dtype=dtype, device=w.device)
    _lib.check(lib.madm_op_pack_linear(_ptr(w), N, K, _ptr(lora_a), _ptr(lora_b), r, scale, _ptr(out), ldo, _dt(out.dtype), _stream()), None,
               "madm_op_pack_linear")
    return out


def pack_conv(w, Cpad=0, out=None, ldo=0, dtype=torch.float16):
    lib = _lib.load()
    N, Cc, kh, kw = w.shape
    taps = kh * kw
    Cpad = Cpad or (Cc + 63) // 64 * 64
    if out is None:
        out = torch.empty(N, taps * Cpad, dtype=dtype, device=w.device)
    _lib.check(lib.madm_op_pack_conv(_ptr(w), N, Cc, taps, Cpad, _ptr(out), ldo, _dt(out.dtype), _stream()), None, "madm_op_pack_conv")
    return out


def pack_conv_dgrad(w, CoPad=0, dtype=torch.float16):
    lib = _lib.load()
    Cout, Cin, kh, kw = w.shape
    taps = kh * kw
    CoPad = CoPad or (Cout + 63) // 64 * 64
    out = torch.empty(Cin, taps * CoPad, dtype=dtype, device=w.device)
    _lib.check(lib.madm_op_pack_conv_dgrad(_ptr(w), Cout, Cin, taps, CoPad, _ptr(out), 0, _dt(dtype), _stream()), None, "madm_op_pack_conv_dgrad")
    return out


def pack_linear_dgrad(w, lora_a=None, lora_b=None, scale=0.0, dtype=torch.float16):
    lib = _lib.load()
    N, K = w.shape
    out = torch.empty(K, N, dtype=dtype, device=w.device)
    r = lora_a.shape[0] if lora_a is not None else 0
    _lib.check(lib.madm_op_pack_linear_dgrad(_ptr(w), N, K, _ptr(lora_a), _ptr(lora_b), r, float(scale), _ptr(out), 0, _dt(dtype), _stream()),
               None, "madm_op_pack_linear_dgrad")
    return out


def pack_geglu(w, bias, dtype=torch.float16):
    lib = _lib.load()
    N2, K = w.shape
    out = torch.empty(N2, K, dtype=dtype, device=w.device)
    ob = torch.empty(N2, dtype=torch.float32, device=w.device)
    _lib.check(lib.madm_op_pack_geglu(_ptr(w), _ptr(bias), N2 // 2, K, _ptr(out), _ptr(ob), _dt(dtype), _stream()), None, "madm_op_pack_geglu")
    return out, ob


def space_to_depth(x, dtype=torch.float16):
    lib = _lib.load()
    B, H, W, Cc = x.shape
    out = torch.empty(4, B, H // 2, W // 2, Cc, dtype=dtype, device=x.device)
    _lib.check(lib.madm_op_space_to_depth(_ptr(x), B, H, W, Cc, _ptr(out), _dt(dtype), _stream()), None, "madm_op_space_to_depth")
    return out


def upsample2x(x, dtype=torch.float16):
    lib = _lib.load()
    B, H, W, Cc = x.shape
    out = torch.empty(B, 2 * H, 2 * W, Cc, dtype=dtype, device=x.device)
    _lib.check(lib.madm_op_upsample2x(_ptr(x), B, H, W, Cc, _ptr(out), _dt(dtype), _stream()), None, "madm_op_upsample2x")
    return out


def nchw_to_nhwc16(x, dtype=torch.float16):
    lib = _lib.load()
    B, Cc, H, W = x.shape
    out = torch.empty(B, H, W, Cc, dtype=dtype, device=x.device)
    _lib.check(lib.madm_op_nchw_to_nhwc16(_ptr(x), B, Cc, H * W, _ptr(out), _dt(dtype), _stream()), None, "madm_op_nchw_to_nhwc16")
    return out


def bilinear_resize(x, Hd, Wd, out=None, pitch=0):
    lib = _lib.load()
    B, Hs, Ws, Cc = x.shape
    if out is None:
        out = torch.empty(B, Hd, Wd, Cc, dtype=x.dtype, device=x.device)
    _lib.check(lib.madm_op_bilinear_resize(_ptr(x), B, Hs, Ws, Cc, _ptr(out), Hd, Wd, pitch or Cc, _dt(x.dtype), _stream()), None,
               "madm_op_bilinear_resize")
    return out


def depthwise3x3(x, w9, shift, dilation):
    lib = _lib.load()
    B, H, W, Cc = x.shape
    out = torch.empty_like(x)
    _lib.check(lib.madm_op_depthwise3x3(_ptr(x), B, H, W, Cc, dilation, _ptr(w9), _ptr(shift), _ptr(out), _dt(x.dtype), _stream()), None,
               "madm_op_depthwise3x3")
    return out


def preprocess_image(img, size, divisibility=64):
    lib = _lib.load()
    x = img.to(torch.float32).contiguous()
    B, Cc, Hs, Ws = x.shape
    Hr, Wr = (Hs, Ws) if size is None else (int(size[0]), int(size[1]))
    Hd, Wd = Hr + (-Hr) % divisibility, Wr + (-Wr) % divisibility
    out = torch.empty(B, Cc, Hd, Wd, dtype=torch.float32, device=x.device)
    _lib.check(lib.madm_op_preprocess_image(_ptr(x), B * Cc, Hs, Ws, Hr, Wr, Hd, Wd, _ptr(out), _stream()), None, "madm_op_preprocess_image")
    return out


def slide_merge(feats, nwin, wins_yx, Hf, Wf):
    lib = _lib.load()
    NB, Cc, hf, wf = feats.shape
    n = NB // nwin
    wins = torch.tensor(list(wins_yx), dtype=torch.int32, device=feats.device).reshape(-1).contiguous()
    out = torch.empty(n, Cc, Hf, Wf, dtype=torch.float32, device=feats.device)
    _lib.check(lib.madm_op_slide_merge(_ptr(feats.contiguous()), nwin, n, Cc, hf, wf, _ptr(wins), Hf, Wf, _ptr(out), _stream()), None,
               "madm_op_slide_merge")
    return out


def image_im2col(img, range_flag=None, dtype=torch.float16):
    lib = _lib.load()
    B, _, H, W = img.shape
    out = torch.empty(B * H * W, 64, dtype=dtype, device=img.device)
    _lib.check(lib.madm_op_image_im2col(_ptr(img), B, H, W, _ptr(out), _ptr(range_flag), _dt(dtype), _stream()), None, "madm_op_image_im2col")
    return out


def gn_add_relu_nchw(a, ga, ba, s, gs, bs, eps, B, HW, Cc):
    lib = _lib.load()
    stats = torch.empty(lib.madm_op_groupnorm_scratch_floats(B, HW, Cc), dtype=torch.float32, device=a.device)
    out = torch.empty(B, Cc, HW, dtype=torch.float32, device=a.device)
    _lib.check(lib.madm_op_gn_add_relu_nchw(_ptr(a), _ptr(ga), _ptr(ba), _ptr(s), _ptr(gs), _ptr(bs), 1 if gs is not None else 0,
                                            eps, B, HW, Cc, _ptr(stats), _ptr(out), _stream()), None, "madm_op_gn_add_relu_nchw")
    return out


def groupnorm_bwd(x0, x1, stats, gamma, beta, eps, act, dy, *, extra=None, want16=True, want32=False, acc=(False, False),
                  dx0=None, dx1=None, want_affine=False):
    lib = _lib.load()
    B, HW, C0 = x0.shape
    C1 = x1.shape[2] if x1 is not None else 0
    Cc = C0 + C1
    dev = x0.device
    in16 = 1 if x0.dtype in (torch.float16, torch.bfloat16) else 0
    scratch = torch.empty(lib.madm_op_groupnorm_bwd_scratch_floats(B, HW, Cc), dtype=torch.float32, device=dev)
    out16 = torch.empty(B, HW, Cc, dtype=dy.dtype, device=dev) if want16 else None
    if want32:
        dx0 = dx0 if dx0 is not None else torch.empty(B, HW, C0, dtype=torch.float32, device=dev)
        if C1:
            dx1 = dx1 if dx1 is not None else torch.empty(B, HW, C1, dtype=torch.float32, device=dev)
    dg = torch.empty(Cc, dtype=torch.float32, device=dev) if want_affine else None
    db = torch.empty(Cc, dtype=torch.float32, device=dev) if want_affine else None
    _lib.check(lib.madm_op_groupnorm_bwd(_ptr(x0), C0, _ptr(x1), C1, B, HW, in16, _ptr(stats), _ptr(gamma), _ptr(beta), float(eps), int(act), _ptr(dy),
                                         _ptr(extra), _ptr(scratch), _ptr(out16), _ptr(dx0), int(acc[0]), _ptr(dx1), int(acc[1]), _ptr(dg), _ptr(db),
                                         _dt(dy.dtype), _stream()), None, "madm_op_groupnorm_bwd")
    return dict(out16=out16, dx0=dx0, dx1=dx1, dgamma=dg, dbeta=db)


def layernorm_bwd(x, gamma, eps, dy, dx=None, accumulate=False):
    lib = _lib.load()
    M, Cc = x.shape
    if dx is None:
        dx = torch.empty(M, Cc, dtype=torch.float32, device=x.device)
    _lib.check(lib.madm_op_layernorm_bwd(_ptr(x), M, Cc, _ptr(gamma), float(eps), _ptr(dy), _ptr(dx), int(accumulate), _dt(dy.dtype), _stream()), None,
               "madm_op_layernorm_bwd")
    return dx


def geglu_fwd(raw):
    lib = _lib.load()
    M, H2 = raw.shape
    out = torch.empty(M, H2 // 2, dtype=raw.dtype, device=raw.device)
    _lib.check(lib.madm_op_geglu_fwd(_ptr(raw), M, H2 // 2, _ptr(out), _dt(raw.dtype), _stream()), None, "madm_op_geglu_fwd")
    return out


def geglu_bwd(raw, dout):
    lib = _lib.load()
    M, H2 = raw.shape
    draw = torch.empty_like(raw)
    _lib.check(lib.madm_op_geglu_bwd(_ptr(raw), _ptr(dout), M, H2 // 2, _ptr(draw), _dt(raw.dtype), _stream()), None, "madm_op_geglu_bwd")
    return draw


def attention_bwd(q, ldq, k, ldk, v, ldv, o, ldo, dout, lddo, dq, lddq, dk, lddk, dv, lddv, B, heads, d, Nq, Nk, q_bs, kv_bs, o_bs, do_bs, dq_bs,
                  dkv_bs, scale):
    lib = _lib.load()
    scratch = torch.empty(lib.madm_op_attention_bwd_scratch_floats(B, heads, d, Nq, Nk), dtype=torch.float32, device=o.device)
    _lib.check(lib.madm_op_attention_bwd(_ptr(q), ldq, _ptr(k), ldk, _ptr(v), ldv, _ptr(o), ldo, _ptr(dout), lddo, _ptr(dq), lddq, _ptr(dk), lddk,
                                         _ptr(dv), lddv, B, heads, d, Nq, Nk, q_bs, kv_bs, o_bs, do_bs, dq_bs, dkv_bs, float(scale), _ptr(scratch),
                                         _dt(o.dtype), _stream()), None, "madm_op_attention_bwd")


def wgrad(dy, x, N, K, *, taps=1, geom=(0, 0, 0), alpha=1.0, transpose_out=False, lda=None, ldb=None, M=None):
    lib = _lib.load()
    M = M if M is not None else dy.shape[0]
    lda = lda if lda is not None else dy.stride(0)
    ldb = ldb if ldb is not None else (x.stride(0) if x.dim() == 2 else x.shape[-1])
    shape = (N, K, 3, 3) if taps == 9 else ((K, N) if transpose_out else (N, K))
    out = torch.empty(shape, dtype=torch.float32, device=dy.device)
    scratch = torch.empty(lib.madm_op_wgrad_scratch_floats(M, N, K, taps), dtype=torch.float32, device=dy.device)
    _lib.check(lib.madm_op_wgrad(_ptr(dy), lda, _ptr(x), ldb, M, N, K, taps, geom[0], geom[1], geom[2], float(alpha), _ptr(out), int(transpose_out),
                                 _ptr(scratch), _dt(dy.dtype), _stream()), None, "madm_op_wgrad")
    return out


def lora_grads(x, dy, A, B, alpha=1.0, M=None, ldx=None, ldy=None):
    lib = _lib.load()
    M = M if M is not None else x.shape[0]
    K, N = A.shape[1], B.shape[0]
    a16 = A.to(x.dtype).contiguous()
    bt16 = B.t().to(x.dtype).contiguous()
    gA = torch.empty(16, K, dtype=torch.float32, device=x.device)
    gB = torch.empty(N, 16, dtype=torch.float32, device=x.device)
    n = lib.madm_op_lora_grads_scratch_floats(M, N, K)
    if n < 0:
        raise ValueError(f"lora_grads: unsupported N / K ({N}, {K})")
    scratch = torch.empty(n, dtype=torch.float32, device=x.device)
    _lib.check(lib.madm_op_lora_grads(_ptr(x), ldx if ldx is not None else x.stride(0), _ptr(dy), ldy if ldy is not None else dy.stride(0), _ptr(a16),
                                      _ptr(bt16), M, N, K, float(alpha), _ptr(gA), _ptr(gB), _ptr(scratch), _dt(x.dtype), _stream()), None,
               "madm_op_lora_grads")
    return gA, gB


def colsum_per_image(x, out=None, col_off=0):
    lib = _lib.load()
    B, HW, Cc = x.shape
    if out is None:
        out = torch.empty(B, Cc, dtype=torch.float32, device=x.device)
    _lib.check(lib.madm_op_colsum_per_image(_ptr(x), B, HW, Cc, C.c_void_p(out.data_ptr() + 4 * col_off), out.stride(0), _dt(x.dtype), _stream()), None,
               "madm_op_colsum_per_image")
    return out


def zero_stuff2x(x):
    lib = _lib.load()
    B, h, w, Cc = x.shape
    out = torch.empty(B, 2 * h, 2 * w, Cc, dtype=x.dtype, device=x.device)
    _lib.check(lib.madm_op_zero_stuff2x(_ptr(x), B, h, w, Cc, _ptr(out), _stream()), None, "madm_op_zero_stuff2x")
    return out


def sum2x2(x, out=None, accumulate=False):
    lib = _lib.load()
    B, H2, W2, Cc = x.shape
    if out is None:
        out = torch.empty(B, H2 // 2, W2 // 2, Cc, dtype=torch.float32, device=x.device)
    _lib.check(lib.madm_op_sum2x2(_ptr(x), B, H2 // 2, W2 // 2, Cc, _ptr(out), int(accumulate), _stream()), None, "madm_op_sum2x2")
    return out


def relu_bwd_nchw(dout, out, scale=1.0, dtype=torch.bfloat16):
    lib = _lib.load()
    B, Cc, H, W = out.shape
    dz = torch.empty(B, H * W, Cc, dtype=dtype, device=out.device)
    _lib.check(lib.madm_op_relu_bwd_nchw(_ptr(dout), _ptr(out), B, Cc, H * W, float(scale), _ptr(dz), _dt(dtype), _stream()), None,
               "madm_op_relu_bwd_nchw")
    return dz
```

Before: 347.9.

## Make tensor-core flash attention persistent for short key sequences

The flash attention kernel can now loop over several (query block, head, batch) work items per CTA. When Nk fits in one key tile, as in the cross-attention over 77 text tokens, the grid is sized to the SM count and each CTA walks a contiguous range of items. A new q_empty barrier lets the producer reload Q once the previous item's S MMAs finish, so TMA loads of the next item can overlap the tail of the current one. The change also adds an LSE-returning attention entry point, reads heads and B from params instead of the grid, and adds more barrier and phase bookkeeping to the kernel.

```diff
diff --git a/include/madm_b200.h b/include/madm_b200.h
--- a/include/madm_b200.h
+++ b/include/madm_b200.h
@@ -159,6 +159,9 @@
                       int32_t B, int32_t heads, int32_t d, int32_t Nq, int32_t Nk, int64_t q_bstride, int64_t kv_bstride,
                       int64_t o_bstride, float scale, int32_t dtype, int32_t impl ,
                       madm_stream stream);
+int madm_op_attention_lse(const void* q, int32_t ldq, const void* k, int32_t ldk, const void* v, int32_t ldv, void* o, int32_t ldo,
+                          int32_t B, int32_t heads, int32_t d, int32_t Nq, int32_t Nk, int64_t q_bstride, int64_t kv_bstride,
+                          int64_t o_bstride, float scale, float* lse, int32_t dtype, madm_stream stream);
 int madm_op_pack_linear(const float* w, int32_t N, int32_t K, const float* lora_a, const float* lora_b, int32_t r, float scale,
                         void* out_bf16, int32_t ldo, int32_t dtype, madm_stream stream);
 int madm_op_pack_conv(const float* w, int32_t N, int32_t C, int32_t taps, int32_t Cpad, void* out_bf16, int32_t ldo,
diff --git a/madm_b200/_lib.py b/madm_b200/_lib.py
--- a/madm_b200/_lib.py
+++ b/madm_b200/_lib.py
@@ -108,6 +108,8 @@
     "madm_op_softmax_rows": (c_int, [c_void_p, c_int32, c_int32, c_void_p, c_int32, c_void_p]),
     "madm_op_attention": (c_int, [c_void_p, c_int32, c_void_p, c_int32, c_void_p, c_int32, c_void_p, c_int32, c_int32,
                                   c_int32, c_int32, c_int32, c_int32, c_int64, c_int64, c_int64, c_float, c_int32, c_int32, c_void_p]),
+    "madm_op_attention_lse": (c_int, [c_void_p, c_int32, c_void_p, c_int32, c_void_p, c_int32, c_void_p, c_int32, c_int32,
+                                      c_int32, c_int32, c_int32, c_int32, c_int64, c_int64, c_int64, c_float, c_void_p, c_int32, c_void_p]),
     "madm_op_pack_linear": (c_int, [c_void_p, c_int32, c_int32, c_void_p, c_void_p, c_int32, c_float, c_void_p, c_int32,
                                     c_int32, c_void_p]),
     "madm_op_pack_conv": (c_int, [c_void_p, c_int32, c_int32, c_int32, c_int32, c_void_p, c_int32, c_int32, c_void_p]),
diff --git a/madm_b200/csrc/api_ops.cu b/madm_b200/csrc/api_ops.cu
--- a/madm_b200/csrc/api_ops.cu
+++ b/madm_b200/csrc/api_ops.cu
@@ -76,6 +76,15 @@
     return fail(e);
   RUN(flash_attention_tc_launch(L, static_cast<cudaStream_t>(stream)));
 }
+int madm_op_attention_lse(const void* q, int32_t ldq, const void* k, int32_t ldk, const void* v, int32_t ldv, void* o, int32_t ldo,
+                          int32_t B, int32_t heads, int32_t d, int32_t Nq, int32_t Nk, int64_t q_bs, int64_t kv_bs, int64_t o_bs,
+                          float scale, float* lse, int32_t dtype, madm_stream stream) {
+  FaLaunch L;
+  if (const char* e = flash_attention_tc_prepare(q, ldq, k, ldk, v, ldv, o, ldo, B, heads, d, Nq, Nk, q_bs, kv_bs, o_bs, scale,
+                                                 dtype == MADM_DTYPE_FP16, &L, lse))
+    return fail(e);
+  RUN(flash_attention_tc_launch(L, static_cast<cudaStream_t>(stream)));
+}
 
 int madm_op_pack_linear(const float* w, int32_t N, int32_t K, const float* la, const float* lb, int32_t r, float scale, void* out,
                         int32_t ldo, int32_t dtype, madm_stream stream) {
diff --git a/madm_b200/csrc/attention_tc.cu b/madm_b200/csrc/attention_tc.cu
--- a/madm_b200/csrc/attention_tc.cu
+++ b/madm_b200/csrc/attention_tc.cu
@@ -46,6 +46,7 @@
   float scale_log2;
   int fp16;
   float* lse;
+  int heads, B;
 };
 
 __device__ __forceinline__ float fa_ex2(float x) {
@@ -54,7 +55,7 @@
   return y;
 }
 
-template <int D, int NQT, bool FP16>
+template <int D, int NQT, bool FP16, bool PERSIST>
 __global__ void __launch_bounds__(FaCfg<D, NQT>::THREADS, 1) fa_tc_kernel(const __grid_constant__ FaParams p) {
   using C = FaCfg<D, NQT>;
   extern __shared__ uint8_t smem_raw[];
@@ -75,15 +76,26 @@
   auto pv_go = [&](int g) { return gbar(g, 4); };
   auto pv_done = [&](int g) { return gbar(g, 5); };
   const uint32_t tmem_slot = sBar + 8u * (9 + 16);
+  const uint32_t q_empty = sBar + 8u * (9 + 17);
   volatile uint32_t* tmem_slot_ptr = reinterpret_cast<volatile uint32_t*>(smem_raw + (tmem_slot - smem_u32(smem_raw)));
 
   const int warp = threadIdx.x >> 5, lane = threadIdx.x & 31;
-  const int q0 = blockIdx.x * (FA_BM * NQT), h = blockIdx.y, b = blockIdx.z;
   const int ntiles = (p.Nk + FA_BN - 1) / FA_BN;
+  const int nqb = (p.Nq + FA_BM * NQT - 1) / (FA_BM * NQT);
+  const int nitems = nqb * p.heads * p.B;
+  const int per = PERSIST ? (nitems + int(gridDim.x) - 1) / int(gridDim.x) : 1;
+  const int it0 = int(blockIdx.x) * per;
+  const int it1 = PERSIST ? min(nitems, it0 + per) : it0 + 1;
+  auto decode = [&](int it, int& q0, int& h, int& b) {
+    q0 = (it % nqb) * (FA_BM * NQT);
+    h = (it / nqb) % p.heads;
+    b = it / (nqb * p.heads);
+  };
 
   if (warp == 0 && lane == 0) {
     prefetch_tmap(&p.tmQ); prefetch_tmap(&p.tmK); prefetch_tmap(&p.tmV);
     mbar_init(q_full, 1);
+    mbar_init(q_empty, NQT);
     for (int s = 0; s < 2; ++s) {
       mbar_init(k_full(s), 1); mbar_init(k_empty(s), NQT); mbar_init(v_full(s), 1); mbar_init(v_empty(s), NQT);
     }
@@ -106,24 +118,29 @@
 
   if (warp == 0) {
     if (elect_one()) {
-      mbar_arrive_expect_tx(q_full, C::Q_BYTES);
-#pragma unroll
-      for (int g = 0; g < NQT; ++g)
-#pragma unroll
-        for (int kc = 0; kc < C::KC; ++kc)
-          tma_load_4d(sQ + (g * C::KC + kc) * FA_TILE, &p.tmQ, q_full, kc * 64, h, q0 + g * FA_BM, b);
       int stage = 0;
       uint32_t phase = 0;
-      for (int j = 0; j < ntiles; ++j) {
-        mbar_wait(k_empty(stage), phase ^ 1u);
-        mbar_arrive_expect_tx(k_full(stage), C::KV_BYTES);
-#pragma unroll
-        for (int kc = 0; kc < C::KC; ++kc) tma_load_4d(sK + stage * C::KV_BYTES + kc * FA_TILE, &p.tmK, k_full(stage), kc * 64, h, j * FA_BN, b);
-        mbar_wait(v_empty(stage), phase ^ 1u);
-        mbar_arrive_expect_tx(v_full(stage), C::KV_BYTES);
-#pragma unroll
-        for (int kc = 0; kc < C::KC; ++kc) tma_load_4d(sV + stage * C::KV_BYTES + kc * FA_TILE, &p.tmV, v_full(stage), kc * 64, h, j * FA_BN, b);
-        if (++stage == C::STAGES) { stage = 0; phase ^= 1u; }
+      for (int it = it0, n = 0; it < it1; ++it, ++n) {
+        int q0, h, b;
+        decode(it, q0, h, b);
+        if (n > 0) mbar_wait(q_empty, (n - 1) & 1);
+        mbar_arrive_expect_tx(q_full, C::Q_BYTES);
+#pragma unroll
+        for (int g = 0; g < NQT; ++g)
+#pragma unroll
+          for (int kc = 0; kc < C::KC; ++kc)
+            tma_load_4d(sQ + (g * C::KC + kc) * FA_TILE, &p.tmQ, q_full, kc * 64, h, q0 + g * FA_BM, b);
+        for (int j = 0; j < ntiles; ++j) {
+          mbar_wait(k_empty(stage), phase ^ 1u);
+          mbar_arrive_expect_tx(k_full(stage), C::KV_BYTES);
+#pragma unroll
+          for (int kc = 0; kc < C::KC; ++kc) tma_load_4d(sK + stage * C::KV_BYTES + kc * FA_TILE, &p.tmK, k_full(stage), kc * 64, h, j * FA_BN, b);
+          mbar_wait(v_empty(stage), phase ^ 1u);
+          mbar_arrive_expect_tx(v_full(stage), C::KV_BYTES);
+#pragma unroll
+          for (int kc = 0; kc < C::KC; ++kc) tma_load_4d(sV + stage * C::KV_BYTES + kc * FA_TILE, &p.tmV, v_full(stage), kc * 64, h, j * FA_BN, b);
+          if (++stage == C::STAGES) { stage = 0; phase ^= 1u; }
+        }
       }
     }
   } else if (warp <= NQT) {
@@ -145,39 +162,45 @@
       pd[1] = make_smem_desc_sw128(sP + (g * 2 + 1) * FA_TILE);
       const uint32_t tmem_og = tmem + C::O_BASE + g * C::O_STRIDE;
       const uint32_t tmem_pg = tmem + C::S_COLS + g * 64;
-      auto issue_s = [&](int j) {
-        const int stage = j % C::STAGES;
-        const int sb = j % C::NSB;
-        mbar_wait(k_full(stage), (j / C::STAGES) & 1);
-        mbar_wait(s_empty(g, sb), ((j / C::NSB) & 1) ^ 1u);
+      auto issue_s = [&](int tb, int j) {
+        const int t = tb + j;
+        const int stage = t % C::STAGES;
+        const int sb = t % C::NSB;
+        mbar_wait(k_full(stage), (t / C::STAGES) & 1);
+        mbar_wait(s_empty(g, sb), ((t / C::NSB) & 1) ^ 1u);
         tc_fence_after();
         const uint32_t ts = tmem + uint32_t((g * C::NSB + sb) * 128);
 #pragma unroll
         for (int ks = 0; ks < C::KSTEPS; ++ks) umma_bf16_ss(ts, qd[ks], stage == 0 ? kd[0][ks] : kd[C::STAGES - 1][ks], idesc_s, ks != 0);
         umma_commit(s_full(g, sb));
         umma_commit(k_empty(stage));
+        if (j == ntiles - 1) umma_commit(q_empty);
       };
-      mbar_wait(q_full, 0);
-      issue_s(0);
-      for (int j = 0; j < ntiles; ++j) {
-        if (j + 1 < ntiles) issue_s(j + 1);
-        const int stage = j % C::STAGES;
-        int keys = p.Nk - j * FA_BN;
-        if (keys > FA_BN) keys = FA_BN;
-        const int ksteps = (keys + 15) >> 4;
-        mbar_wait(pv_go(g), j & 1);
-        tc_fence_after();
-        const uint64_t vds = stage == 0 ? vd[0] : vd[C::STAGES - 1];
-#pragma unroll
-        for (int kk = 0; kk < FA_BN / 16; ++kk) {
-          if (kk < ksteps) {
-            const uint64_t bd = vds + uint64_t(kk * (2048 >> 4));
-            if constexpr (C::P_TMEM) umma_f16_ts(tmem_og, tmem_pg + kk * 8, bd, idesc_o, kk != 0);
-            else umma_bf16_ss(tmem_og, pd[kk >> 2] + uint64_t(2 * (kk & 3)), bd, idesc_o, kk != 0);
-          }
+      for (int it = it0, n = 0; it < it1; ++it, ++n) {
+        const int tb = n * ntiles;
+        mbar_wait(q_full, n & 1);
+        issue_s(tb, 0);
+        for (int j = 0; j < ntiles; ++j) {
+          if (j + 1 < ntiles) issue_s(tb, j + 1);
+          const int t = tb + j;
+          const int stage = t % C::STAGES;
+          int keys = p.Nk - j * FA_BN;
+          if (keys > FA_BN) keys = FA_BN;
+          const int ksteps = (keys + 15) >> 4;
+          mbar_wait(pv_go(g), t & 1);
+          tc_fence_after();
+          const uint64_t vds = stage == 0 ? vd[0] : vd[C::STAGES - 1];
+#pragma unroll
+          for (int kk = 0; kk < FA_BN / 16; ++kk) {
+            if (kk < ksteps) {
+              const uint64_t bd = vds + uint64_t(kk * (2048 >> 4));
+              if constexpr (C::P_TMEM) umma_f16_ts(tmem_og, tmem_pg + kk * 8, bd, idesc_o, kk != 0);
+              else umma_bf16_ss(tmem_og, pd[kk >> 2] + uint64_t(2 * (kk & 3)), bd, idesc_o, kk != 0);
+            }
+          }
+          umma_commit(pv_done(g));
+          umma_commit(v_empty(stage));
         }
-        umma_commit(pv_done(g));
-        umma_commit(v_empty(stage));
       }
     }
   } else {
@@ -191,94 +214,176 @@
     const float sl = p.scale_log2;
     constexpr int fp16 = FP16 ? 1 : 0;
     constexpr int OC = C::ONES ? D + 1 : D;
-    float o_acc[C::DV];
-#pragma unroll
-    for (int i = 0; i < C::DV; ++i) o_acc[i] = 0.f;
-    float m_run = -INFINITY, l_run = 0.f, corr_prev = 1.f;
     uint32_t r[32];
-
-    auto o_update = [&](float corr) {
-      tc_fence_after();
-      constexpr int OB = (C::DV % 48 == 0) ? 48 : 32;
-#pragma unroll
-      for (int c0 = 0; c0 < C::DV; c0 += OB) {
-        uint32_t ro[OB];
-        __syncwarp();
-        if (c0 + 0 < C::DV) tmem_ld16_at<0>(tmem_o + c0, ro);
-        if (c0 + 16 < C::DV) tmem_ld16_at<16>(tmem_o + c0 + 16, ro);
-        if constexpr (OB == 48) { if (c0 + 32 < C::DV) tmem_ld16_at<32>(tmem_o + c0 + 32, ro); }
-        tmem_ld_wait();
-#pragma unroll
-        for (int i = 0; i < OB; ++i)
-          if (c0 + i < OC) o_acc[c0 + i] = fmaf(o_acc[c0 + i], corr, __uint_as_float(ro[i]));
-      }
-      tc_fence_before();
-    };
-
-    for (int j = 0; j < ntiles; ++j) {
-      const int sb = j % C::NSB;
-      mbar_wait(s_full(g, sb), (j / C::NSB) & 1);
-      tc_fence_after();
-      const uint32_t ts = tmem + lane_base + uint32_t((g * C::NSB + sb) * 128);
-      const int kvalid = p.Nk - j * FA_BN;
-      const bool ragged = kvalid < FA_BN;
-      float corr, rs = 0.f;
-      if constexpr (C::REG_S && C::P_TMEM) {
-        uint32_t sc[4][32];
-        __syncwarp();
-#pragma unroll
-        for (int c = 0; c < 4; ++c) tmem_ld32(ts + c * 32, sc[c]);
-        tmem_ld_wait();
+    for (int it = it0, tb = 0; it < it1; ++it, tb += ntiles) {
+      float o_acc[C::DV];
+#pragma unroll
+      for (int i = 0; i < C::DV; ++i) o_acc[i] = 0.f;
+      float m_run = -INFINITY, l_run = 0.f, corr_prev = 1.f;
+
+      auto o_update = [&](float corr) {
+        tc_fence_after();
+        constexpr int OB = (C::DV % 48 == 0) ? 48 : 32;
+#pragma unroll
+        for (int c0 = 0; c0 < C::DV; c0 += OB) {
+          uint32_t ro[OB];
+          __syncwarp();
+          if (c0 + 0 < C::DV) tmem_ld16_at<0>(tmem_o + c0, ro);
+          if (c0 + 16 < C::DV) tmem_ld16_at<16>(tmem_o + c0 + 16, ro);
+          if constexpr (OB == 48) { if (c0 + 32 < C::DV) tmem_ld16_at<32>(tmem_o + c0 + 32, ro); }
+          tmem_ld_wait();
+#pragma unroll
+          for (int i = 0; i < OB; ++i)
+            if (c0 + i < OC) o_acc[c0 + i] = fmaf(o_acc[c0 + i], corr, __uint_as_float(ro[i]));
+        }
         tc_fence_before();
-        __syncwarp();
-        if (lane == 0) mbar_arrive(s_empty(g, sb));
-        if (ragged) {
-#pragma unroll
-          for (int c = 0; c < 4; ++c)
-#pragma unroll
-            for (int i = 0; i < 32; ++i)
-              if (c * 32 + i >= kvalid) sc[c][i] = 0xff800000u;
-        }
-        float mx0 = m_run, mx1 = -INFINITY, mx2 = -INFINITY, mx3 = -INFINITY;
-#pragma unroll
-        for (int i = 0; i < 32; ++i) {
-          mx0 = fmaxf(mx0, __uint_as_float(sc[0][i]));
-          mx1 = fmaxf(mx1, __uint_as_float(sc[1][i]));
-          mx2 = fmaxf(mx2, __uint_as_float(sc[2][i]));
-          mx3 = fmaxf(mx3, __uint_as_float(sc[3][i]));
-        }
-        const float mx = fmaxf(fmaxf(mx0, mx1), fmaxf(mx2, mx3));
-        corr = fa_ex2((m_run - mx) * sl);
-        m_run = mx;
-        const float ms = -mx * sl;
-        {
-          const int stage = j % C::STAGES;
-          mbar_wait(v_full(stage), (j / C::STAGES) & 1);
-          if constexpr (C::ONES) {
-            const uint32_t addr = sV + stage * C::KV_BYTES + uint32_t(D >> 6) * FA_TILE + uint32_t(row) * 128 +
-                                  uint32_t((((D & 63) >> 3) ^ (row & 7)) << 4) + uint32_t((D & 7) * 2);
-            const uint16_t one = FP16 ? 0x3C00 : 0x3F80;
-            asm volatile("st.shared.u16 [%0], %1;" ::"r"(addr), "h"(one) : "memory");
-          }
-        }
-        float rs1 = 0.f;
-#pragma unroll
-        for (int c = 0; c < 4; ++c) {
-          uint32_t pk[16];
-#pragma unroll
-          for (int i = 0; i < 32; i += 2) {
-            const float p0 = fa_ex2(fmaf(__uint_as_float(sc[c][i]), sl, ms));
-            const float p1 = fa_ex2(fmaf(__uint_as_float(sc[c][i + 1]), sl, ms));
-            pk[i >> 1] = pack2_16(p0, p1, fp16);
-            if constexpr (!C::ONES) { rs += p0; rs1 += p1; }
-          }
-          if (c == 0) {
-            if (j > 0) mbar_wait(pv_done(g), (j - 1) & 1);
-            if constexpr (C::P_TMEM) { tc_fence_after(); __syncwarp(); }
-          }
-          if constexpr (C::P_TMEM) {
-            tmem_st16(tmem_p + c * 16, pk);
-          } else {
+      };
+
+      for (int j = 0; j < ntiles; ++j) {
+        const int t = tb + j;
+        const int sb = t % C::NSB;
+        mbar_wait(s_full(g, sb), (t / C::NSB) & 1);
+        tc_fence_after();
+        const uint32_t ts = tmem + lane_base + uint32_t((g * C::NSB + sb) * 128);
+        const int kvalid = p.Nk - j * FA_BN;
+        const bool ragged = kvalid < FA_BN;
+        float corr, rs = 0.f;
+        if constexpr (C::REG_S && C::P_TMEM) {
+          uint32_t sc[4][32];
+          __syncwarp();
+#pragma unroll
+          for (int c = 0; c < 4; ++c) tmem_ld32(ts + c * 32, sc[c]);
+          tmem_ld_wait();
+          tc_fence_before();
+          __syncwarp();
+          if (lane == 0) mbar_arrive(s_empty(g, sb));
+          if (ragged) {
+#pragma unroll
+            for (int c = 0; c < 4; ++c)
+#pragma unroll
+              for (int i = 0; i < 32; ++i)
+                if (c * 32 + i >= kvalid) sc[c][i] = 0xff800000u;
+          }
+          float mx0 = m_run, mx1 = -INFINITY, mx2 = -INFINITY, mx3 = -INFINITY;
+#pragma unroll
+          for (int i = 0; i < 32; ++i) {
+            mx0 = fmaxf(mx0, __uint_as_float(sc[0][i]));
+            mx1 = fmaxf(mx1, __uint_as_float(sc[1][i]));
+            mx2 = fmaxf(mx2, __uint_as_float(sc[2][i]));
+            mx3 = fmaxf(mx3, __uint_as_float(sc[3][i]));
+          }
+          const float mx = fmaxf(fmaxf(mx0, mx1), fmaxf(mx2, mx3));
+          corr = fa_ex2((m_run - mx) * sl);
+          m_run = mx;
+          const float ms = -mx * sl;
+          {
+            const int stage = t % C::STAGES;
+            mbar_wait(v_full(stage), (t / C::STAGES) & 1);
+            if constexpr (C::ONES) {
+              const uint32_t addr = sV + stage * C::KV_BYTES + uint32_t(D >> 6) * FA_TILE + uint32_t(row) * 128 +
+                                    uint32_t((((D & 63) >> 3) ^ (row & 7)) << 4) + uint32_t((D & 7) * 2);
+              const uint16_t one = FP16 ? 0x3C00 : 0x3F80;
+              asm volatile("st.shared.u16 [%0], %1;" ::"r"(addr), "h"(one) : "memory");
+            }
+          }
+          float rs1 = 0.f;
+#pragma unroll
+          for (int c = 0; c < 4; ++c) {
+            uint32_t pk[16];
+#pragma unroll
+            for (int i = 0; i < 32; i += 2) {
+              const float p0 = fa_ex2(fmaf(__uint_as_float(sc[c][i]), sl, ms));
+              const float p1 = fa_ex2(fmaf(__uint_as_float(sc[c][i + 1]), sl, ms));
+              pk[i >> 1] = pack2_16(p0, p1, fp16);
+              if constexpr (!C::ONES) { rs += p0; rs1 += p1; }
+            }
+            if (c == 0) {
+              if (j > 0) mbar_wait(pv_done(g), (t - 1) & 1);
+              if constexpr (C::P_TMEM) { tc_fence_after(); __syncwarp(); }
+            }
+            if constexpr (C::P_TMEM) {
+              tmem_st16(tmem_p + c * 16, pk);
+            } else {
+              const uint32_t chunk_base = sPg + uint32_t(c >> 1) * FA_TILE + uint32_t(row) * 128;
+              const int u0 = (c & 1) * 4;
+#pragma unroll
+              for (int u = 0; u < 4; ++u) {
+                const uint32_t addr = chunk_base + uint32_t(((u0 + u) ^ (row & 7)) << 4);
+                asm volatile("st.shared.v4.b32 [%0], {%1,%2,%3,%4};" ::"r"(addr), "r"(pk[4 * u]), "r"(pk[4 * u + 1]), "r"(pk[4 * u + 2]),
+                             "r"(pk[4 * u + 3]) : "memory");
+              }
+            }
+          }
+          if constexpr (C::P_TMEM) { tmem_st_wait(); tc_fence_before(); }
+          rs += rs1;
+        } else if constexpr (C::REG_S) {
+          uint32_t sa[32], sb2[32];
+          float mx0 = m_run, mx1 = -INFINITY, mx2 = -INFINITY, mx3 = -INFINITY;
+#pragma unroll
+          for (int hlf = 0; hlf < 2; ++hlf) {
+            __syncwarp();
+            tmem_ld32(ts + hlf * 64, sa);
+            tmem_ld32(ts + hlf * 64 + 32, sb2);
+            tmem_ld_wait();
+            if (ragged) {
+#pragma unroll
+              for (int i = 0; i < 32; ++i) {
+                if (hlf * 64 + i >= kvalid) sa[i] = 0xff800000u;
+                if (hlf * 64 + 32 + i >= kvalid) sb2[i] = 0xff800000u;
+              }
+            }
+#pragma unroll
+            for (int i = 0; i < 32; i += 2) {
+              mx0 = fmaxf(mx0, __uint_as_float(sa[i]));
+              mx1 = fmaxf(mx1, __uint_as_float(sa[i + 1]));
+              mx2 = fmaxf(mx2, __uint_as_float(sb2[i]));
+              mx3 = fmaxf(mx3, __uint_as_float(sb2[i + 1]));
+            }
+          }
+          const float mx = fmaxf(fmaxf(mx0, mx1), fmaxf(mx2, mx3));
+          corr = fa_ex2((m_run - mx) * sl);
+          m_run = mx;
+          const float ms = -mx * sl;
+          {
+            const int stage = t % C::STAGES;
+            mbar_wait(v_full(stage), (t / C::STAGES) & 1);
+            if constexpr (C::ONES) {
+              const uint32_t addr = sV + stage * C::KV_BYTES + uint32_t(D >> 6) * FA_TILE + uint32_t(row) * 128 +
+                                    uint32_t((((D & 63) >> 3) ^ (row & 7)) << 4) + uint32_t((D & 7) * 2);
+              const uint16_t one = FP16 ? 0x3C00 : 0x3F80;
+              asm volatile("st.shared.u16 [%0], %1;" ::"r"(addr), "h"(one) : "memory");
+            }
+          }
+          float rs1 = 0.f;
+          __syncwarp();
+          tmem_ld32(ts, sa);
+#pragma unroll
+          for (int c = 0; c < 4; ++c) {
+            uint32_t (&cur)[32] = (c & 1) ? sb2 : sa;
+            uint32_t (&nxt)[32] = (c & 1) ? sa : sb2;
+            tmem_ld_wait();
+            if (c < 3) {
+              __syncwarp();
+              tmem_ld32(ts + (c + 1) * 32, nxt);
+            } else {
+              tc_fence_before();
+              __syncwarp();
+              if (lane == 0) mbar_arrive(s_empty(g, sb));
+            }
+            if (ragged) {
+#pragma unroll
+              for (int i = 0; i < 32; ++i)
+                if (c * 32 + i >= kvalid) cur[i] = 0xff800000u;
+            }
+            uint32_t pk[16];
+#pragma unroll
+            for (int i = 0; i < 32; i += 2) {
+              const float p0 = fa_ex2(fmaf(__uint_as_float(cur[i]), sl, ms));
+              const float p1 = fa_ex2(fmaf(__uint_as_float(cur[i + 1]), sl, ms));
+              pk[i >> 1] = pack2_16(p0, p1, fp16);
+              if constexpr (!C::ONES) { rs += p0; rs1 += p1; }
+            }
+            if (c == 0 && j > 0) mbar_wait(pv_done(g), (t - 1) & 1);
             const uint32_t chunk_base = sPg + uint32_t(c >> 1) * FA_TILE + uint32_t(row) * 128;
             const int u0 = (c & 1) * 4;
 #pragma unroll
@@ -288,160 +393,83 @@
                            "r"(pk[4 * u + 3]) : "memory");
             }
           }
+          rs += rs1;
+        } else {
+          float mx = m_run;
+#pragma unroll 1
+          for (int c = 0; c < FA_BN; c += 32) {
+            __syncwarp();
+            tmem_ld32(ts + c, r);
+            tmem_ld_wait();
+            if (c + 32 <= kvalid) {
+#pragma unroll
+              for (int i = 0; i < 32; ++i) mx = fmaxf(mx, __uint_as_float(r[i]));
+            } else {
+#pragma unroll
+              for (int i = 0; i < 32; ++i)
+                if (c + i < kvalid) mx = fmaxf(mx, __uint_as_float(r[i]));
+            }
+          }
+          corr = fa_ex2((m_run - mx) * sl);
+          m_run = mx;
+          const float ms = -mx * sl;
+          mbar_wait(v_full(t % C::STAGES), (t / C::STAGES) & 1);
+          if (j > 0) mbar_wait(pv_done(g), (t - 1) & 1);
+#pragma unroll 1
+          for (int c = 0; c < FA_BN; c += 32) {
+            __syncwarp();
+            tmem_ld32(ts + c, r);
+            tmem_ld_wait();
+            uint32_t pk[16];
+#pragma unroll
+            for (int i = 0; i < 32; i += 2) {
+              float p0 = fa_ex2(fmaf(__uint_as_float(r[i]), sl, ms));
+              float p1 = fa_ex2(fmaf(__uint_as_float(r[i + 1]), sl, ms));
+              if (c + i >= kvalid) p0 = 0.f;
+              if (c + i + 1 >= kvalid) p1 = 0.f;
+              rs += p0 + p1;
+              pk[i >> 1] = pack2_16(p0, p1, fp16);
+            }
+            const uint32_t chunk_base = sPg + uint32_t(c >> 6) * FA_TILE + uint32_t(row) * 128;
+            const int u0 = (c & 63) >> 3;
+#pragma unroll
+            for (int u = 0; u < 4; ++u) {
+              const uint32_t addr = chunk_base + uint32_t(((u0 + u) ^ (row & 7)) << 4);
+              asm volatile("st.shared.v4.b32 [%0], {%1,%2,%3,%4};" ::"r"(addr), "r"(pk[4 * u]), "r"(pk[4 * u + 1]), "r"(pk[4 * u + 2]),
+                           "r"(pk[4 * u + 3]) : "memory");
+            }
+          }
+          tc_fence_before();
+          __syncwarp();
+          if (lane == 0) mbar_arrive(s_empty(g, sb));
         }
-        if constexpr (C::P_TMEM) { tmem_st_wait(); tc_fence_before(); }
-        rs += rs1;
-      } else if constexpr (C::REG_S) {
-        uint32_t sa[32], sb2[32];
-        float mx0 = m_run, mx1 = -INFINITY, mx2 = -INFINITY, mx3 = -INFINITY;
-#pragma unroll
-        for (int hlf = 0; hlf < 2; ++hlf) {
-          __syncwarp();
-          tmem_ld32(ts + hlf * 64, sa);
-          tmem_ld32(ts + hlf * 64 + 32, sb2);
-          tmem_ld_wait();
-          if (ragged) {
-#pragma unroll
-            for (int i = 0; i < 32; ++i) {
-              if (hlf * 64 + i >= kvalid) sa[i] = 0xff800000u;
-              if (hlf * 64 + 32 + i >= kvalid) sb2[i] = 0xff800000u;
-            }
-          }
-#pragma unroll
-          for (int i = 0; i < 32; i += 2) {
-            mx0 = fmaxf(mx0, __uint_as_float(sa[i]));
-            mx1 = fmaxf(mx1, __uint_as_float(sa[i + 1]));
-            mx2 = fmaxf(mx2, __uint_as_float(sb2[i]));
-            mx3 = fmaxf(mx3, __uint_as_float(sb2[i + 1]));
-          }
-        }
-        const float mx = fmaxf(fmaxf(mx0, mx1), fmaxf(mx2, mx3));
-        corr = fa_ex2((m_run - mx) * sl);
-        m_run = mx;
-        const float ms = -mx * sl;
-        {
-          const int stage = j % C::STAGES;
-          mbar_wait(v_full(stage), (j / C::STAGES) & 1);
-          if constexpr (C::ONES) {
-            const uint32_t addr = sV + stage * C::KV_BYTES + uint32_t(D >> 6) * FA_TILE + uint32_t(row) * 128 +
-                                  uint32_t((((D & 63) >> 3) ^ (row & 7)) << 4) + uint32_t((D & 7) * 2);
-            const uint16_t one = FP16 ? 0x3C00 : 0x3F80;
-            asm volatile("st.shared.u16 [%0], %1;" ::"r"(addr), "h"(one) : "memory");
-          }
-        }
-        float rs1 = 0.f;
-        __syncwarp();
-        tmem_ld32(ts, sa);
-#pragma unroll
-        for (int c = 0; c < 4; ++c) {
-          uint32_t (&cur)[32] = (c & 1) ? sb2 : sa;
-          uint32_t (&nxt)[32] = (c & 1) ? sa : sb2;
-          tmem_ld_wait();
-          if (c < 3) {
-            __syncwarp();
-            tmem_ld32(ts + (c + 1) * 32, nxt);
-          } else {
-            tc_fence_before();
-            __syncwarp();
-            if (lane == 0) mbar_arrive(s_empty(g, sb));
-          }
-          if (ragged) {
-#pragma unroll
-            for (int i = 0; i < 32; ++i)
-              if (c * 32 + i >= kvalid) cur[i] = 0xff800000u;
-          }
-          uint32_t pk[16];
-#pragma unroll
-          for (int i = 0; i < 32; i += 2) {
-            const float p0 = fa_ex2(fmaf(__uint_as_float(cur[i]), sl, ms));
-            const float p1 = fa_ex2(fmaf(__uint_as_float(cur[i + 1]), sl, ms));
-            pk[i >> 1] = pack2_16(p0, p1, fp16);
-            if constexpr (!C::ONES) { rs += p0; rs1 += p1; }
-          }
-          if (c == 0 && j > 0) mbar_wait(pv_done(g), (j - 1) & 1);
-          const uint32_t chunk_base = sPg + uint32_t(c >> 1) * FA_TILE + uint32_t(row) * 128;
-          const int u0 = (c & 1) * 4;
-#pragma unroll
-          for (int u = 0; u < 4; ++u) {
-            const uint32_t addr = chunk_base + uint32_t(((u0 + u) ^ (row & 7)) << 4);
-            asm volatile("st.shared.v4.b32 [%0], {%1,%2,%3,%4};" ::"r"(addr), "r"(pk[4 * u]), "r"(pk[4 * u + 1]), "r"(pk[4 * u + 2]),
-                         "r"(pk[4 * u + 3]) : "memory");
-          }
-        }
-        rs += rs1;
-      } else {
-        float mx = m_run;
-#pragma unroll 1
-        for (int c = 0; c < FA_BN; c += 32) {
-          __syncwarp();
-          tmem_ld32(ts + c, r);
-          tmem_ld_wait();
-          if (c + 32 <= kvalid) {
-#pragma unroll
-            for (int i = 0; i < 32; ++i) mx = fmaxf(mx, __uint_as_float(r[i]));
-          } else {
-#pragma unroll
-            for (int i = 0; i < 32; ++i)
-              if (c + i < kvalid) mx = fmaxf(mx, __uint_as_float(r[i]));
-          }
-        }
-        corr = fa_ex2((m_run - mx) * sl);
-        m_run = mx;
-        const float ms = -mx * sl;
-        mbar_wait(v_full(j % C::STAGES), (j / C::STAGES) & 1);
-        if (j > 0) mbar_wait(pv_done(g), (j - 1) & 1);
-#pragma unroll 1
-        for (int c = 0; c < FA_BN; c += 32) {
-          __syncwarp();
-          tmem_ld32(ts + c, r);
-          tmem_ld_wait();
-          uint32_t pk[16];
-#pragma unroll
-          for (int i = 0; i < 32; i += 2) {
-            float p0 = fa_ex2(fmaf(__uint_as_float(r[i]), sl, ms));
-            float p1 = fa_ex2(fmaf(__uint_as_float(r[i + 1]), sl, ms));
-            if (c + i >= kvalid) p0 = 0.f;
-            if (c + i + 1 >= kvalid) p1 = 0.f;
-            rs += p0 + p1;
-            pk[i >> 1] = pack2_16(p0, p1, fp16);
-          }
-          const uint32_t chunk_base = sPg + uint32_t(c >> 6) * FA_TILE + uint32_t(row) * 128;
-          const int u0 = (c & 63) >> 3;
-#pragma unroll
-          for (int u = 0; u < 4; ++u) {
-            const uint32_t addr = chunk_base + uint32_t(((u0 + u) ^ (row & 7)) << 4);
-            asm volatile("st.shared.v4.b32 [%0], {%1,%2,%3,%4};" ::"r"(addr), "r"(pk[4 * u]), "r"(pk[4 * u + 1]), "r"(pk[4 * u + 2]),
-                         "r"(pk[4 * u + 3]) : "memory");
-          }
-        }
+        l_run = l_run * corr + rs;
+        fence_proxy_async();
+        if (j > 0) o_update(corr_prev);
+        corr_prev = corr;
         tc_fence_before();
         __syncwarp();
-        if (lane == 0) mbar_arrive(s_empty(g, sb));
+        if (lane == 0) mbar_arrive(pv_go(g));
       }
-      l_run = l_run * corr + rs;
-      fence_proxy_async();
-      if (j > 0) o_update(corr_prev);
-      corr_prev = corr;
-      tc_fence_before();
-      __syncwarp();
-      if (lane == 0) mbar_arrive(pv_go(g));
-    }
-    mbar_wait(pv_done(g), (ntiles - 1) & 1);
-    o_update(corr_prev);
-    const int m = q0 + g * FA_BM + row;
-    if (m < p.Nq) {
-      const float den = C::ONES ? o_acc[C::ONES ? D : 0] : l_run;
-      const float inv = 1.0f / den;
-      if (p.lse) p.lse[(size_t(b) * gridDim.y + h) * p.Nq + m] = (m_run * p.scale_log2 + log2f(den)) * 0.6931471805599453f;
-      uint16_t* op = p.O + size_t(b) * p.o_bs + size_t(m) * p.ldo + h * D;
-#pragma unroll
-      for (int c = 0; c < D; c += 8) {
-        uint4 v;
-        v.x = pack2_16(o_acc[c] * inv, o_acc[c + 1] * inv, fp16);
-        v.y = pack2_16(o_acc[c + 2] * inv, o_acc[c + 3] * inv, fp16);
-        v.z = pack2_16(o_acc[c + 4] * inv, o_acc[c + 5] * inv, fp16);
-        v.w = pack2_16(o_acc[c + 6] * inv, o_acc[c + 7] * inv, fp16);
-        *reinterpret_cast<uint4*>(op + c) = v;
+      mbar_wait(pv_done(g), (tb + ntiles - 1) & 1);
+      o_update(corr_prev);
+      int q0, h, b;
+      decode(it, q0, h, b);
+      const int m = q0 + g * FA_BM + row;
+      if (m < p.Nq) {
+        const float den = C::ONES ? o_acc[C::ONES ? D : 0] : l_run;
+        const float inv = 1.0f / den;
+        if (p.lse) p.lse[(size_t(b) * p.heads + h) * p.Nq + m] = (m_run * p.scale_log2 + log2f(den)) * 0.6931471805599453f;
+        uint16_t* op = p.O + size_t(b) * p.o_bs + size_t(m) * p.ldo + h * D;
+#pragma unroll
+        for (int c = 0; c < D; c += 8) {
+          uint4 v;
+          v.x = pack2_16(o_acc[c] * inv, o_acc[c + 1] * inv, fp16);
+          v.y = pack2_16(o_acc[c + 2] * inv, o_acc[c + 3] * inv, fp16);
+          v.z = pack2_16(o_acc[c + 4] * inv, o_acc[c + 5] * inv, fp16);
+          v.w = pack2_16(o_acc[c + 6] * inv, o_acc[c + 7] * inv, fp16);
+          *reinterpret_cast<uint4*>(op + c) = v;
+        }
       }
     }
   }
@@ -507,26 +535,39 @@
   p->lse = lse;
   L->d = d;
   L->nqt = (d <= 80 && Nq >= 2 * FA_BM) ? 2 : 1;
-  L->grid = dim3((Nq + FA_BM * L->nqt - 1) / (FA_BM * L->nqt), heads, B);
+  p->heads = heads;
+  p->B = B;
+  const int nitems = (Nq + FA_BM * L->nqt - 1) / (FA_BM * L->nqt) * heads * B;
+  int ctas = nitems;
+  if (Nk <= FA_BN) {
+    int dev = 0, sms = 0;
+    if (cudaGetDevice(&dev) != cudaSuccess || cudaDeviceGetAttribute(&sms, cudaDevAttrMultiProcessorCount, dev) != cudaSuccess || sms < 1)
+      return "attention: cannot query the SM count";
+    const int per = (nitems + sms - 1) / sms;
+    ctas = (nitems + per - 1) / per;
+  }
+  L->grid = dim3(ctas);
   return nullptr;
 }
 
-template <int D, int NQT, bool FP16>
+template <int D, int NQT, bool FP16, bool PERSIST>
 static const char* fa_launch_t(const FaLaunch& L, cudaStream_t st) {
   using C = FaCfg<D, NQT>;
   static bool attr = false;
   if (!attr) {
-    if (cudaFuncSetAttribute(fa_tc_kernel<D, NQT, FP16>, cudaFuncAttributeMaxDynamicSharedMemorySize, int(C::SMEM)) != cudaSuccess)
+    if (cudaFuncSetAttribute(fa_tc_kernel<D, NQT, FP16, PERSIST>, cudaFuncAttributeMaxDynamicSharedMemorySize, int(C::SMEM)) != cudaSuccess)
       return "attention: cudaFuncSetAttribute failed";
     attr = true;
   }
-  if (launch_k(fa_tc_kernel<D, NQT, FP16>, L.grid, dim3(C::THREADS), C::SMEM, st, *reinterpret_cast<const FaParams*>(L.params)) != cudaSuccess)
+  if (launch_k(fa_tc_kernel<D, NQT, FP16, PERSIST>, L.grid, dim3(C::THREADS), C::SMEM, st, *reinterpret_cast<const FaParams*>(L.params)) != cudaSuccess)
     return "fa_tc launch failed";
   return cudaGetLastError() == cudaSuccess ? nullptr : "attention: launch failed";
 }
 template <int D, int NQT>
 static const char* fa_launch_d(const FaLaunch& L, cudaStream_t st) {
-  return reinterpret_cast<const FaParams*>(L.params)->fp16 ? fa_launch_t<D, NQT, true>(L, st) : fa_launch_t<D, NQT, false>(L, st);
+  const FaParams& p = *reinterpret_cast<const FaParams*>(L.params);
+  if (p.Nk <= FA_BN) return p.fp16 ? fa_launch_t<D, NQT, true, true>(L, st) : fa_launch_t<D, NQT, false, true>(L, st);
+  return p.fp16 ? fa_launch_t<D, NQT, true, false>(L, st) : fa_launch_t<D, NQT, false, false>(L, st);
 }
 
 const char* flash_attention_tc_launch(const FaLaunch& L, cudaStream_t st) {
diff --git a/madm_b200/ops.py b/madm_b200/ops.py
--- a/madm_b200/ops.py
+++ b/madm_b200/ops.py
@@ -123,6 +123,14 @@
                                      o_bs, scale, _dt(o.dtype), impl, _stream()), None, "madm_op_attention")
 
 
+def attention_lse(q, ldq, k, ldk, v, ldv, o, ldo, B, heads, d, Nq, Nk, q_bs, kv_bs, o_bs, scale):
+    lib = _lib.load()
+    lse = torch.empty(B, heads, Nq, dtype=torch.float32, device=o.device)
+    _lib.check(lib.madm_op_attention_lse(_ptr(q), ldq, _ptr(k), ldk, _ptr(v), ldv, _ptr(o), ldo, B, heads, d, Nq, Nk, q_bs, kv_bs,
+                                         o_bs, scale, _ptr(lse), _dt(o.dtype), _stream()), None, "madm_op_attention_lse")
+    return lse
+
+
 def pack_linear(w, lora_a=None, lora_b=None, scale=0.0, out=None, ldo=0, dtype=torch.float16):
     lib = _lib.load()
     N, K = w.shape
```

Result: no change. 349.5 (median of 6 runs) (+0.4%).
